# Spockuto/drand

Hardware: AMD Instinct MI355X
Metric: beacons verified/s (batch chain verify) (higher is better)
Workload: dtype u32 (381-bit Montgomery, 12x32-bit limbs); 1 GPU; configs[1]: 1000000-round chained beacon history per GPU, chain.VerifyBeacon per round; beacons_per_gpu=1000000, segment_len=64, parallelism=range-shard x1

## Files before the change

### drand_amd/_lib.py

```python
from __future__ import annotations

import ctypes
import os

_HERE = os.path.dirname(os.path.abspath(__file__))
LIB_PATH = os.environ.get("DRAND_AMD_LIB", os.path.join(_HERE, "libblsverify.so"))

BLSV_OK = 0
BLSV_EINVAL = -1
BLSV_EHIP = -2
BLSV_ENOGROUP = -3
BLSV_ENOTENOUGH = -4

AGG_OK = 0
AGG_OK_V2 = 1
AGG_V1_RECOVER_FAIL = 2
AGG_V1_INVALID = 3
AGG_V2_RECOVER_FAIL = 4

REJ_OK = 0
REJ_LENGTH = 1
REJ_FLAG = 2
REJ_INF_NONZERO = 3
REJ_X_GE_P = 4
REJ_NOT_ON_CURVE = 5
REJ_NOT_IN_SUBGROUP = 6
REJ_PAIRING = 7
REJ_SHARE_INDEX = 8

REJ_NAMES = {
    REJ_OK: "ok",
    REJ_LENGTH: "bad length",
    REJ_FLAG: "bad compression flag",
    REJ_INF_NONZERO: "infinity with non-zero bits",
    REJ_X_GE_P: "coordinate >= p",
    REJ_NOT_ON_CURVE: "point is not on curve",
    REJ_NOT_IN_SUBGROUP: "point is not on correct subgroup",
    REJ_PAIRING: "bls: invalid signature",
    REJ_SHARE_INDEX: "tbls: invalid signature share",
}

u8p = ctypes.POINTER(ctypes.c_uint8)
u32p = ctypes.POINTER(ctypes.c_uint32)
u64p = ctypes.POINTER(ctypes.c_uint64)
vp = ctypes.c_void_p
sz = ctypes.c_size_t

SIGNATURES = {
    "blsv_version": (ctypes.c_char_p, []),
    "blsv_device_count": (ctypes.c_int, []),
    "blsv_create": (ctypes.c_int, [ctypes.c_int, ctypes.POINTER(vp)]),
    "blsv_destroy": (None, [vp]),
    "blsv_last_error": (ctypes.c_char_p, [vp]),
    "blsv_synchronize": (ctypes.c_int, [vp]),
    "blsv_set_group": (ctypes.c_int, [vp, u8p, sz, sz]),
    "blsv_verify_chained": (ctypes.c_int, [vp, ctypes.c_uint64, u8p, sz, u8p, sz, u8p, u64p, u8p]),
    "blsv_verify_chained_multi": (ctypes.c_int, [ctypes.POINTER(vp), sz, ctypes.POINTER(sz), ctypes.c_uint64, u8p, sz,
                                                  u8p, sz, u8p, u64p, u8p]),
    "blsv_verify_prevs": (ctypes.c_int, [vp, ctypes.c_uint64, u8p, sz, u8p, sz, u8p, u64p, u8p]),
    "blsv_verify_unchained": (ctypes.c_int, [vp, u64p, ctypes.c_uint64, u8p, sz, u8p, u64p, u8p]),
    "blsv_verify_messages": (ctypes.c_int, [vp, u8p, u8p, u32p, sz, u8p, u8p, u64p, u8p]),
    "blsv_verify_partials": (ctypes.c_int, [vp, u8p, sz, u8p, sz, sz, u8p, u8p]),
    "blsv_verify_partials_multi": (ctypes.c_int, [vp, u8p, u32p, u8p, sz, sz, u8p, u8p]),
    "blsv_recover": (ctypes.c_int, [vp, u8p, sz, u8p, sz, sz, sz, sz, u8p]),
    "blsv_aggregate": (ctypes.c_int, [vp, u8p, sz, u8p, sz, sz, sz, sz, u8p, u8p, u8p, u8p]),
    "blsv_aggregate_round": (ctypes.c_int, [vp, u8p, sz, u8p, sz, u8p, sz, u8p, sz, sz, sz, sz, u8p, u8p, u8p, u8p,
                                             ctypes.POINTER(ctypes.c_int32), u8p]),
    "blsv_sign": (ctypes.c_int, [vp, u8p, ctypes.c_int32, u8p, u32p, sz, u8p]),
    "blsv_verify_chained_dev": (ctypes.c_int, [vp, ctypes.c_uint64, ctypes.c_uint64, ctypes.c_uint64, vp, sz, vp, sz,
                                                vp, vp, vp, vp]),
    "blsv_generate_chained_dev": (ctypes.c_int, [vp, u8p, ctypes.c_uint64, ctypes.c_uint64, vp, sz, vp, sz, vp]),
    "blsv_profile_enable": (ctypes.c_int, [vp, ctypes.c_int]),
    "blsv_profile_read": (ctypes.c_int, [vp, ctypes.POINTER(ctypes.c_double), u64p, u64p, ctypes.c_int]),
    "blsv_lat_trace": (ctypes.c_int, [vp, u64p, ctypes.c_int, ctypes.POINTER(ctypes.c_double), ctypes.c_int]),
    "blsv_test_fp_mul": (ctypes.c_int, [vp, u32p, u32p, sz, u32p]),
    "blsv_test_op": (ctypes.c_int, [vp, ctypes.c_char_p, u32p, sz, u32p]),
    "blsv_test_op_info": (ctypes.c_int, [ctypes.c_int, ctypes.POINTER(ctypes.c_char_p), ctypes.POINTER(ctypes.c_int),
                                         ctypes.POINTER(ctypes.c_int), ctypes.POINTER(ctypes.c_int)]),
    "blsv_test_pairing": (ctypes.c_int, [vp, u32p, u32p, sz, u32p]),
    "blsv_test_hash_to_g2": (ctypes.c_int, [vp, u8p, u32p, sz, u32p, u8p]),
    "blsv_test_final_exp": (ctypes.c_int, [vp, u32p, sz, u32p, u32p]),
    "blsv_test_tail_split": (ctypes.c_int, [vp, sz]),
    "blsv_set_lat_max": (sz, [vp, sz]),
    "blsv_set_chunk": (sz, [vp, sz]),
    "blsv_workspace_bytes": (sz, [vp]),
    "blsv_lat_trace_enable": (ctypes.c_int, [vp, ctypes.c_int]),
    "blsv_test_generic_chains": (ctypes.c_int, [vp, ctypes.c_int]),
    "blsv_test_spec_stats": (ctypes.c_int, [vp, ctypes.POINTER(ctypes.c_uint64), ctypes.POINTER(ctypes.c_uint64)]),
    "blsv_test_lagrange": (ctypes.c_int, [ctypes.POINTER(ctypes.c_uint32), ctypes.c_size_t, ctypes.POINTER(ctypes.c_uint32)]),
    "blsv_service_create": (ctypes.c_int, [ctypes.c_int, ctypes.c_uint32, ctypes.c_uint32, ctypes.POINTER(vp)]),
    "blsv_service_destroy": (None, [vp]),
    "blsv_service_verify_partial": (ctypes.c_int, [vp, u8p, sz, sz, u8p, sz, u8p, sz, u8p, u8p]),
    "blsv_service_verify_recovered": (ctypes.c_int, [vp, u8p, u8p, sz, u8p, u8p, u8p]),
    "blsv_service_stats": (ctypes.c_int, [vp, u64p, u64p, u64p]),
    "blsv_test_service_limits": (ctypes.c_int, [vp, sz, sz, sz, u64p]),
    "blsv_verify_chained_rlc": (ctypes.c_int, [vp, ctypes.c_uint64, u8p, sz, u8p, sz, u8p, u64p, u8p]),
    "blsv_verify_unchained_rlc": (ctypes.c_int, [vp, u64p, ctypes.c_uint64, u8p, sz, u8p, u64p, u8p]),
    "blsv_verify_chained_rlc_dev": (ctypes.c_int, [vp, ctypes.c_uint64, ctypes.c_uint64, ctypes.c_uint64, vp, sz, vp,
                                                    sz, vp, vp, vp, vp]),
    "blsv_set_rlc_group": (sz, [vp, sz]),
    "blsv_rlc_stats": (ctypes.c_int, [vp, u64p, u64p, u64p]),
    "blsv_test_rlc_seed": (ctypes.c_int, [vp, u8p]),
    "blsv_test_rlc_sums": (ctypes.c_int, [vp, ctypes.c_uint64, u8p, sz, u8p, sz, u8p, u8p]),
    "blsv_tlock_open": (ctypes.c_int, [vp, u8p, u8p, sz, u8p, u8p, u8p, u8p]),
    "blsv_tlock_open_dev": (ctypes.c_int, [vp, u8p, vp, sz, vp, vp, vp]),
    "blsv_tlock_stats": (ctypes.c_int, [vp, u64p, u64p]),
    "blsv_tlock_seal": (ctypes.c_int, [vp, u8p, ctypes.c_uint64, u8p, sz, u8p, u8p, u8p]),
    "blsv_tlock_seal_dev": (ctypes.c_int, [vp, u8p, ctypes.c_uint64, vp, sz, vp, vp, vp, vp]),
    "blsv_tlock_seal_stats": (ctypes.c_int, [vp, u64p, u64p]),
}

_lib = None


class EngineUnavailable(RuntimeError):
    """The HIP engine library could not be loaded (no silent fallback exists)."""


def load():
    global _lib
    if _lib is not None:
        return _lib
    if not os.path.exists(LIB_PATH):
        raise EngineUnavailable(
            f"{LIB_PATH} not found: build it with `python -c 'import __graft_entry__ as g; g.build()'` "
            "(make -C drand_amd/csrc); drand_amd has no CPU fallback")
    try:
        lib = ctypes.CDLL(LIB_PATH)
    except OSError as e:
        raise EngineUnavailable(f"cannot load {LIB_PATH}: {e}") from e
    for name, (res, args) in SIGNATURES.items():
        fn = getattr(lib, name)
        fn.restype = res
        fn.argtypes = args
    _lib = lib
    return lib


def buf(data):
    if data is None:
        return None
    b = bytes(data)
    arr = (ctypes.c_uint8 * max(len(b), 1)).from_buffer_copy(b if b else b"\0")
    return arr


def out_buf(n):
    return (ctypes.c_uint8 * max(n, 1))()
```

### drand_amd/csrc/blsverify.cpp

```cpp
#include "host_internal.h"

void release_workspace(blsv_ctx* c) {
  for (DBuf* d : {&c->H, &c->HQ, &c->S, &c->F, &c->FW, &c->LN, &c->h_inf, &c->s_inf, &c->cls}) d->release();
  c->cap = 0;
}

int ensure_workspace(blsv_ctx* c, size_t cnt) {
  for (;;) {
    size_t want = std::min(std::max(cnt, size_t(64)), c->chunk);
    want = (want + 63) & ~size_t(63);
    if (want <= c->cap) return BLSV_OK;
    hipError_t e = hipSuccess;
    auto need = [&](DBuf& d, size_t bytes) {
      if (e == hipSuccess) e = d.ensure(bytes);
    };
    need(c->H, want * blsk::H_WORDS * 4);
    need(c->HQ, kHqWords(want) * 4);
    need(c->S, want * blsk::S_WORDS * 4);
    need(c->F, want * blsk::F_WORDS * 4);
    need(c->FW, 3 * want * blsk::F_WORDS * 4);
    need(c->LN, std::max(std::min(want, kLineSub) * blsk::MILLER_LINE_WORDS, blsk::FEXP_PARK_WORDS(want)) * 4);
    need(c->h_inf, want);
    need(c->s_inf, want);
    need(c->cls, want);
    static_assert(3 * blsk::F_WORDS >= 48 * 64 / 21 + 1, "FW holds the Miller park of a sub-chunk");
    if (e == hipSuccess) {
      c->cap = want;
      return BLSV_OK;
    }
    release_workspace(c);
    (void)hipGetLastError();
    if (e != hipErrorOutOfMemory || want <= kMinChunk)
      return fail(c, BLSV_EHIP, "staging for %zu items: %s", want, hipGetErrorString(e));
    c->chunk = std::max(kMinChunk, ((want / 2) + 63) & ~size_t(63));
    c->lat_max = std::min(c->lat_max, c->chunk);
    c->oom_halvings++;
  }
}

hipError_t h2d(blsv_ctx* c, void* dst, const void* src, size_t len) {
  if (!len) return hipSuccess;
  if (len > kIoCap / 4) return hipMemcpyAsync(dst, src, len, hipMemcpyHostToDevice, c->stream);
  if (!c->io_up.p) {
    hipError_t e = c->io_up.ensure(kIoCap);
    if (e != hipSuccess) return e;
  }
  if (c->io_up_off + len > kIoCap) {
    hipError_t e = hipStreamSynchronize(c->stream);
    if (e != hipSuccess) return e;
    c->io_up_off = 0;
  }
  uint8_t* h = c->io_up.as<uint8_t>() + c->io_up_off;
  memcpy(h, src, len);
  c->io_up_off += (len + 63) & ~size_t(63);
  return hipMemcpyAsync(dst, h, len, hipMemcpyHostToDevice, c->stream);
}

hipError_t download_sync(blsv_ctx* c, std::initializer_list<Down> ds) {
  size_t total = 0;
  for (const Down& d : ds) total += (d.len + 63) & ~size_t(63);
  const bool staged = total <= kIoCap && (c->io_down.p || c->io_down.ensure(kIoCap) == hipSuccess);
  hipError_t e = hipSuccess;
  size_t off = 0;
  for (const Down& d : ds) {
    if (!d.len) continue;
    void* to = staged ? (void*)(c->io_down.as<uint8_t>() + off) : d.user;
    if (e == hipSuccess) e = hipMemcpyAsync(to, d.dev, d.len, hipMemcpyDeviceToHost, c->stream);
    off += (d.len + 63) & ~size_t(63);
  }
  const hipError_t es = hipStreamSynchronize(c->stream);
  if (e == hipSuccess) e = es;
  if (e == hipSuccess) c->io_up_off = 0;
  if (e != hipSuccess || !staged) return e;
  off = 0;
  for (const Down& d : ds) {
    if (d.len) memcpy(d.user, c->io_down.as<uint8_t>() + off, d.len);
    off += (d.len + 63) & ~size_t(63);
  }
  return hipSuccess;
}

hipEvent_t take_event(blsv_ctx* c) {
  if (!c->event_pool.empty()) {
    hipEvent_t e = c->event_pool.back();
    c->event_pool.pop_back();
    return e;
  }
  hipEvent_t e = nullptr;
  if (hipEventCreate(&e) != hipSuccess) return nullptr;
  return e;
}

extern "C" {

const char* blsv_version(void) { return "drand_amd blsverify 0.1 (gfx950)"; }

int blsv_device_count(void) {
  int n = 0;
  return hipGetDeviceCount(&n) == hipSuccess ? n : 0;
}

int blsv_create(int device, blsv_ctx** out) {
  if (!out) return BLSV_EINVAL;
  *out = nullptr;
  blsv_ctx* c = new blsv_ctx();
  c->device = device;
  hipError_t e = hipSetDevice(device);
  if (e == hipSuccess) e = hipStreamCreateWithFlags(&c->stream, hipStreamNonBlocking);
  if (e == hipSuccess) e = hipStreamCreateWithFlags(&c->side, hipStreamNonBlocking);
  if (e == hipSuccess) e = hipStreamCreateWithFlags(&c->side2, hipStreamNonBlocking);
  for (hipEvent_t& ev : c->hash_ev)
    if (e == hipSuccess) e = hipEventCreateWithFlags(&ev, hipEventDisableTiming);
  if (e == hipSuccess) e = hipEventCreateWithFlags(&c->fork_ev, hipEventDisableTiming);
  if (e == hipSuccess) e = hipEventCreateWithFlags(&c->join_ev, hipEventDisableTiming);
  int cus = 0;
  if (e == hipSuccess) e = hipDeviceGetAttribute(&cus, hipDeviceAttributeMultiprocessorCount, device);
  c->tail_q_dev = c->tail_q = size_t(64) * 4 * (size_t)std::max(cus, 0);
  if (e != hipSuccess) {
    fprintf(stderr, "blsv_create: %s\n", hipGetErrorString(e));
    blsv_destroy(c);
    return BLSV_EHIP;
  }
  *out = c;
  return BLSV_OK;
}

void blsv_destroy(blsv_ctx* c) {
  if (!c) return;
  (void)hipSetDevice(c->device);
  for (hipStream_t s : {c->stream, c->side, c->side2}) {
    if (!s) continue;
    (void)hipStreamSynchronize(s);
    (void)hipStreamDestroy(s);
  }
  for (hipEvent_t ev : c->hash_ev)
    if (ev) (void)hipEventDestroy(ev);
  if (c->fork_ev) (void)hipEventDestroy(c->fork_ev);
  if (c->join_ev) (void)hipEventDestroy(c->join_ev);
  (void)hipDeviceSynchronize();
  for (auto& r : c->recs)
    for (hipEvent_t e : {r.a, r.b, r.a2, r.b2})
      if (e) (void)hipEventDestroy(e);
  for (auto e : c->event_pool) (void)hipEventDestroy(e);
  delete c;
}

const char* blsv_last_error(const blsv_ctx* c) { return c ? c->err.c_str() : "null context"; }

int blsv_synchronize(blsv_ctx* c) {
  if (!c) return BLSV_EINVAL;
  HIPCHK(c, hipStreamSynchronize(c->stream));
  return BLSV_OK;
}

int blsv_profile_enable(blsv_ctx* c, int on) {
  if (!c) return BLSV_EINVAL;
  c->prof = on != 0;
  return BLSV_OK;
}

int blsv_profile_read(blsv_ctx* c, double* ms, uint64_t* launches, uint64_t* items, int nstages) {
  if (!c || nstages < 0) return BLSV_EINVAL;
  (void)hipSetDevice(c->device);
  for (int s = 0; s < nstages; s++) {
    if (ms) ms[s] = 0;
    if (launches) launches[s] = 0;
    if (items) items[s] = 0;
  }
  for (auto& r : c->recs) {
    HIPCHK(c, hipEventSynchronize(r.b));
    float t = 0;
    HIPCHK(c, hipEventElapsedTime(&t, r.a, r.b));
    if (r.a2 && r.b2) {
      float t2 = 0;
      HIPCHK(c, hipEventSynchronize(r.b2));
      HIPCHK(c, hipEventElapsedTime(&t2, r.a2, r.b2));
      t += t2;
    }
    if (r.stage < nstages) {
      if (ms) ms[r.stage] += t;
      if (launches) launches[r.stage] += 1;
      if (items) items[r.stage] += r.items;
    }
    for (hipEvent_t e : {r.a, r.b, r.a2, r.b2})
      if (e) c->event_pool.push_back(e);
  }
  c->recs.clear();
  return ST_N;
}

size_t blsv_set_lat_max(blsv_ctx* c, size_t lat_max) {
  if (!c) return 0;
  const size_t prev = c->lat_max;
  c->lat_max = std::min(lat_max, c->chunk);
  return prev;
}

size_t blsv_set_chunk(blsv_ctx* c, size_t items) {
  if (!c) return 0;
  const size_t prev = c->chunk;
  size_t v = items ? std::min(std::max(items, kMinChunk), kMaxChunk) : chunk_env();
  v = (v + 63) & ~size_t(63);
  (void)hipSetDevice(c->device);
  if (v < c->cap) {
    (void)hipStreamSynchronize(c->stream);
    (void)hipStreamSynchronize(c->side);
    release_workspace(c);
  }
  c->chunk = v;
  c->lat_max = std::min(c->lat_max, v);
  return prev;
}

size_t blsv_workspace_bytes(const blsv_ctx* c) {
  if (!c) return 0;
  size_t b = 0;
  for (const DBuf* d : {&c->H, &c->HQ, &c->S, &c->F, &c->FW, &c->LN, &c->h_inf, &c->s_inf, &c->cls}) b += d->sz;
  return b;
}

}
```

### drand_amd/csrc/engine_ctx.h

```cpp
#pragma once
#include <hip/hip_runtime.h>

#include <algorithm>
#include <cerrno>
#include <cstdarg>
#include <cstdio>
#include <cstdlib>
#include <cstring>
#include <string>
#include <vector>

#include "../../include/blsverify.h"
#include "kernels.h"

namespace blsv_detail {

constexpr size_t kMaxChunk = size_t(1) << 20;
constexpr size_t kMinChunk = size_t(1) << 14;
constexpr size_t kLineSub = kMaxChunk;
constexpr size_t kPkTable = 4096;
constexpr size_t kFexpParkWords(size_t items) { return blsk::FEXP_PARK_WORDS(items) + 48 * 64; }
constexpr size_t kHqWords(size_t items) { return std::max(items * blsk::HQ_WORDS, kFexpParkWords(items)); }
constexpr size_t kStagingBytesPerItem =
    4 * (blsk::H_WORDS + blsk::HQ_WORDS + 3 + blsk::S_WORDS + 4 * blsk::F_WORDS + blsk::MILLER_LINE_WORDS) + 3;
// ... 2 lines not shown
static_assert((133ull * kMaxChunk) * 4 < 0xffffffffull, "SoA VGPR byte offset exceeds 32 bits");
static_assert(48ull * 4 * kMaxChunk < 0x7fffffffull, "3-lane park slot resource exceeds 31 bits");
static_assert(blsk::G1_WORDS <= blsk::H_WORDS, "timelock: the U table does not fit the H staging");
static_assert(blsk::F_WORDS <= blsk::HQ_WORDS, "timelock: the captured Fp12 does not fit the HQ staging");
static_assert(BLSV_GT_LEN == 4 * blsk::F_WORDS, "timelock: the Gt encoding is one F staging row per item");
static_assert(BLSV_U_LEN <= 4 * blsk::S_WORDS, "timelock: a host call's compressed U bytes do not fit the S staging");
static_assert(BLSV_SCALAR_LEN <= 4 * blsk::S_WORDS, "sealing: a host call's scalars do not fit the S staging");
static_assert(BLSV_U_LEN <= 4 * blsk::H_WORDS, "sealing: the compressed U bytes do not fit the H staging");
static_assert(blsk::G1_WORDS <= blsk::S_WORDS, "sealing: the decoded key does not fit the S staging");
static_assert(blsk::FEXP_PARK_WORDS(1) + blsk::kTlockTabWords <= 64 * blsk::MILLER_LINE_WORDS,
              "sealing: the base's line table does not fit LN behind the park (the smallest workspace is 64 items)");

struct DBuf {
  void* p = nullptr;
  size_t sz = 0;
  ~DBuf() {
    if (p) (void)hipFree(p);
  }
  void release() {
    if (p) (void)hipFree(p);
    p = nullptr;
    sz = 0;
  }
  hipError_t ensure(size_t need) {
    if (need <= sz) return hipSuccess;
    if (p) {
      (void)hipFree(p);
      p = nullptr;
      sz = 0;
    }
    size_t want = std::max(need, size_t(256));
    hipError_t e = hipMalloc(&p, want);
    if (e == hipSuccess) sz = want;
    return e;
  }
  template <typename T>
  T* as() const {
    return static_cast<T*>(p);
  }
};

struct PinBuf {
  void* p = nullptr;
  size_t sz = 0;
  ~PinBuf() {
    if (p) (void)hipHostFree(p);
  }
  hipError_t ensure(size_t need) {
    if (need <= sz) return hipSuccess;
    if (p) (void)hipHostFree(p);
    p = nullptr;
    sz = 0;
    const size_t want = std::max(need + need / 2, size_t(4096));
    hipError_t e = hipHostMalloc(&p, want, hipHostMallocDefault);
    if (e == hipSuccess) sz = want;
    return e;
  }
  template <typename T>
  T* as() const {
    return static_cast<T*>(p);
  }
};

}
using namespace blsv_detail;

enum Stage {
  ST_HASH = 0,
  ST_DECOMP = 1,
  ST_MILLER = 2,
  ST_FEXP = 3,
  ST_FINISH = 4,
  ST_LAT = 5,
  ST_RLC = 6,
  ST_TLOCK = 7,
  ST_N = 8
};
struct ProfRec {
  int stage;
  size_t items;
  hipEvent_t a, b;
  hipEvent_t a2 = nullptr, b2 = nullptr;
};

constexpr size_t kRlcGroupDefault = 64;
constexpr size_t kRlcGroupMin = 8, kRlcGroupMax = 4096;
constexpr size_t kLatMaxDefault = 1536;
inline size_t chunk_env() {
  static const size_t v = [] {
    const char* e = getenv("BLSV_CHUNK");
    if (!e) return kMaxChunk;
    char* end = nullptr;
    errno = 0;
    const unsigned long long x = strtoull(e, &end, 10);
    if (end == e || *end != '\0' || errno == ERANGE || e[0] == '-' || x == 0) {
      fprintf(stderr, "blsverify: ignoring BLSV_CHUNK=\"%s\" (not a positive integer); chunk stays %zu\n", e, kMaxChunk);
      return kMaxChunk;
    }
    const size_t c = (size_t)std::min<unsigned long long>(std::max<unsigned long long>(x, kMinChunk), kMaxChunk);
    return (c + 63) & ~size_t(63);
  }();
  return v;
}

inline size_t lat_max_env() {
  static const size_t v = [] {
    const char* e = getenv("BLSV_LAT_MAX");
    if (!e) return kLatMaxDefault;
    char* end = nullptr;
    errno = 0;
    const unsigned long long x = strtoull(e, &end, 10);
    if (end == e || *end != '\0' || errno == ERANGE || e[0] == '-') {
      fprintf(stderr, "blsverify: ignoring BLSV_LAT_MAX=\"%s\" (not a non-negative integer); cutover stays %zu\n", e,
              kLatMaxDefault);
      return kLatMaxDefault;
    }
    return (size_t)std::min<unsigned long long>(x, kMaxChunk);
  }();
  return v;
}

struct rlc_state {
  size_t group = kRlcGroupDefault;
  bool seed_pinned = false;
  uint8_t seed[32] = {0};
  uint64_t groups = 0, groups_failed = 0, items_exact = 0;
  DBuf part, gH, gS, g_hinf, g_sinf, gcls, cH, cS, c_hinf, c_sinf, ccls, fail, out96;
  PinBuf host;
};

struct tlock_state {
  bool valid = false;
  uint8_t sig[96] = {0};
  uint8_t cls = 0;
  uint64_t prepared = 0, items = 0;
  DBuf d_sig, S, s_inf, s_cls, tab;
};

struct tseal_state {
  bool valid = false, t1_built = false;
  uint8_t pk[48] = {0};
  uint64_t round = 0;
  uint64_t bases = 0, items = 0;
  DBuf t1, t2;
};

struct blsv_ctx {
  int device = 0;
  bool prof = false;
  size_t chunk = chunk_env();
  size_t lat_max = std::min(lat_max_env(), chunk);
  uint64_t oom_halvings = 0;
  size_t tail_q_dev = 0, tail_q = 0;
  std::vector<ProfRec> recs;
  std::vector<hipEvent_t> event_pool;
  hipStream_t stream = nullptr;
  hipStream_t side = nullptr;
  hipEvent_t fork_ev = nullptr, join_ev = nullptr;
  hipStream_t side2 = nullptr;
  hipEvent_t hash_ev[2] = {nullptr, nullptr};
  std::string err;
  bool has_group = false;
  size_t t = 0, n = 0;
  DBuf commits, commit_inf;
  std::vector<uint8_t> group_bytes;
  DBuf pk_all, pk_all_inf;
  size_t pk_all_n = 0;
  bool pk_all_built = false;
  DBuf pk_tab, pk_inf;
  uint8_t pk_cache[48];
  bool pk_cache_valid = false;
  size_t cap = 0;
  DBuf H, S, F, FW, LN, h_inf, s_inf, cls;
  DBuf HQ;
  DBuf in_sigs, in_msgs, in_off, in_len, in_rounds, seeds, bitmap, first_bad, sk, idx, lambdas, scratch, out,
      pp_tab, pp_inf, sel, g1_cls, misc;
  PinBuf pin;
  PinBuf io_up, io_down;
  size_t io_up_off = 0;
  struct SpecSlot {
    DBuf sig, S, s_inf, cls, sel, lam, scratch, out, vmsg, voff, vlen, vcls;
    DBuf hout, saff;
    PinBuf host;
  } spec[2];
  uint64_t spec_hits = 0, spec_misses = 0;
  DBuf arena;
  rlc_state rlc;
  tlock_state tlock;
  tseal_state tseal;
};

#define HIPCHK(ctx, expr)                                                             \
  do {                                                                                \
    hipError_t e_ = (expr);                                                           \
    if (e_ != hipSuccess) return fail((ctx), BLSV_EHIP, "%s: %s", #expr, hipGetErrorString(e_)); \
  } while (0)

inline int fail(blsv_ctx* ctx, int code, const char* fmt, ...) {
  char buf[512];
  va_list ap;
  va_start(ap, fmt);
  vsnprintf(buf, sizeof buf, fmt, ap);
  va_end(ap);
  if (ctx) ctx->err = buf;
  return code;
}


int ensure_workspace(blsv_ctx* c, size_t cnt);
void release_workspace(blsv_ctx* c);

int svc_verify_mixed(blsv_ctx* c, size_t n, const uint8_t* msgs, const uint64_t* off, const uint32_t* lens,
                     const uint8_t* sigs96, const uint32_t* idx, const uint32_t* d_tab, const uint8_t* d_tab_inf,
                     uint8_t* cls_out);
```

### drand_amd/csrc/fp.h

```cpp
#pragma once
#include <stdint.h>
#include "bls_constants.h"

#ifdef BLS_HOST
#include <stddef.h>
#define DI inline
#define NOINL static inline
namespace bls {
extern unsigned long long g_fp_mul_count;
}
#define BLS_COUNT_MUL() (++::bls::g_fp_mul_count)
#else
#include <hip/hip_runtime.h>
#define DI __device__ __forceinline__
#define NOINL static __device__ __noinline__
#define BLS_COUNT_MUL() ((void)0)
#endif

namespace bls {

struct fp {
  uint32_t l[12];
};

// ... 603 lines not shown

DI fp fp_pow_sqrt_inv(const fp& a) { return fp_from_u12(fp_pow_p_minus_3_div_4(fp_to_u12(a))); }


DI int fp_bitlen12(const uint32_t (&c)[12]) {
  int n = 0;
#pragma unroll
  for (int i = 0; i < 12; i++) n = c[i] ? 32 * i + 32 - __builtin_clz(c[i]) : n;
  return n;
}

DI uint64_t fp_top33(const uint32_t (&x)[12], int s) {
  const int w = s >> 5, o = s & 31;
  uint32_t x0 = 0, x1 = 0;
#pragma unroll
  for (int i = 0; i < 12; i++) {
    x0 = i == w ? x[i] : x0;
    x1 = i == w + 1 ? x[i] : x1;
  }
  return ((((uint64_t)x1 << 32) | x0) >> o) & ((1ull << 33) - 1);
}

DI int64_t fp_lincomb28(const uint32_t (&X)[14], const uint32_t (&Y)[14], int64_t f, int64_t g,
                        uint32_t (&L)[14]) {
  int64_t acc = 0;
#pragma unroll
  for (int k = 0; k < 14; k++) {
    acc += (int64_t)X[k] * f + (int64_t)Y[k] * g;
    L[k] = (uint32_t)acc & M28;
    acc >>= 28;
  }
  return acc;
}

DI void fp_lincomb_shr31(const uint32_t (&X)[14], const uint32_t (&Y)[14], int64_t f, int64_t g, uint32_t (&r)[12],
                         bool& neg) {
  uint32_t L[16];
  uint32_t L14[14];
  const int64_t top = fp_lincomb28(X, Y, f, g, L14);
#pragma unroll
  for (int k = 0; k < 14; k++) L[k] = L14[k];
  L[14] = (uint32_t)top & M28;
  L[15] = (uint32_t)(top >> 28) & M28;
#pragma unroll
  for (int j = 0; j < 12; j++) {
    const int B = 31 + 32 * j, k = B / 28, o = B % 28;
    uint64_t v = ((uint64_t)L[k] >> o) | ((uint64_t)L[k + 1] << (28 - o));
    if (k + 2 < 16) v |= (uint64_t)L[k + 2] << (56 - o);
    r[j] = (uint32_t)v;
  }
  neg = top < 0;
  const uint32_t m = neg ? 0xffffffffu : 0u;
  unsigned c = neg ? 1u : 0u;
#pragma unroll
  for (int j = 0; j < 12; j++) r[j] = __builtin_addc(r[j] ^ m, 0u, c, &c);
}

DI fp fp_lincomb_mont56(const uint32_t (&X)[14], const uint32_t (&Y)[14], int64_t f, int64_t g) {
  uint32_t m[2], L[14];
  int64_t acc = 0;
#pragma unroll
  for (int k = 0; k < 16; k++) {
    if (k < 14) acc += (int64_t)X[k] * f + (int64_t)Y[k] * g;
#pragma unroll
    for (int j = 0; j < 2; j++)
      if (j < k && k - j < 14) acc += (int64_t)m[j] * P28[k - j];
    if (k < 2) {
      m[k] = ((uint32_t)acc * P_INV28) & M28;
      acc += (int64_t)m[k] * P28[0];
      acc >>= 28;
    } else {
      L[k - 2] = (uint32_t)acc & M28;
      acc >>= 28;
    }
  }
  const u12 w = fp_join28(L);
  const uint32_t msk = acc < 0 ? 0xffffffffu : 0u;
  fp r;
  unsigned c = 0;
#pragma unroll
  for (int i = 0; i < 12; i++) r.l[i] = __builtin_addc(w[i], P2_RAW[i] & msk, c, &c);
  return r;
}

DI u12 fp_inv_bingcd_raw(u12 yin, bool& converged) {
  uint32_t a[12], b[12];
  const fp yc = fp_canon(fp_from_u12(yin));
#pragma unroll
  for (int i = 0; i < 12; i++) {
    a[i] = yc.l[i];
    b[i] = P_RAW[i];
  }
  fp u = fp_zero(), v = fp_zero();
  u.l[0] = 1;
#pragma unroll 1
  for (int it = 0; it < 25; it++) {
    uint32_t c[12];
#pragma unroll
    for (int i = 0; i < 12; i++) c[i] = a[i] | b[i];
    const int n0 = fp_bitlen12(c), n = n0 > 64 ? n0 : 64;
    uint64_t A = ((uint64_t)(a[0] & 0x7fffffffu)) | (fp_top33(a, n - 33) << 31);
    uint64_t B = ((uint64_t)(b[0] & 0x7fffffffu)) | (fp_top33(b, n - 33) << 31);
    int64_t f0 = 1, g0 = 0, f1 = 0, g1 = 1;
#pragma unroll
    for (int j = 0; j < 31; j++) {
      const bool odd = (A & 1u) != 0;
      const bool sw = odd & (A < B);
      const uint64_t A2 = sw ? B : A, B2 = sw ? A : B;
      const int64_t F0 = sw ? f1 : f0, G0 = sw ? g1 : g0, F1 = sw ? f0 : f1, G1 = sw ? g0 : g1;
      A = odd ? A2 - B2 : A2;
      f0 = odd ? F0 - F1 : F0;
      g0 = odd ? G0 - G1 : G0;
      B = B2;
      f1 = F1;
      g1 = G1;
      A >>= 1;
      f1 = (int64_t)((uint64_t)f1 << 1);
      g1 = (int64_t)((uint64_t)g1 << 1);
    }
    uint32_t X[14], Y[14];
    u12 av, bv;
#pragma unroll
    for (int i = 0; i < 12; i++) av[i] = a[i], bv[i] = b[i];
    fp_split28(av, X);
    fp_split28(bv, Y);
    bool na, nb;
    fp_lincomb_shr31(X, Y, f0, g0, a, na);
    fp_lincomb_shr31(X, Y, f1, g1, b, nb);
    f0 = na ? -f0 : f0;
    g0 = na ? -g0 : g0;
    f1 = nb ? -f1 : f1;
    g1 = nb ? -g1 : g1;
    fp_split28(fp_to_u12(u), X);
    fp_split28(fp_to_u12(v), Y);
    u = fp_lincomb_mont56(X, Y, f0, g0);
    v = fp_lincomb_mont56(X, Y, f1, g1);
  }
  uint32_t nb = b[0] ^ 1u;
#pragma unroll
  for (int i = 1; i < 12; i++) nb |= b[i];
  converged = (nb == 0) | fp_raw_is_zero(yc);
  return fp_to_u12(fp_mul(v, fp_load_const(FP_INV_FIX)));
}

NOINL u12 fp_inv_bingcd(u12 yin) {
  bool ok;
  u12 r = fp_inv_bingcd_raw(yin, ok);
  if (!ok) r = fp_pow_p_minus_2(yin);
  return r;
}

DI fp fp_inv(const fp& a) { return fp_from_u12(fp_inv_bingcd(fp_to_u12(a))); }

DI fp fp_sqrt_cand(const fp& a) { return fp_from_u12(fp_pow_sqrt(fp_to_u12(a))); }

DI bool fp_is_square(const fp& a) {
  fp l = fp_from_u12(fp_pow_legendre(fp_to_u12(a)));
  return fp_is_zero(l) || fp_eq(l, fp_one());
}

DI fp fp_raw_from_be48(const uint8_t* b) {
  fp r;
#pragma unroll
  for (int i = 0; i < 12; i++) {
    const uint8_t* q = b + 44 - 4 * i;
    r.l[i] = ((uint32_t)q[0] << 24) | ((uint32_t)q[1] << 16) | ((uint32_t)q[2] << 8) | (uint32_t)q[3];
  }
  return r;
}

DI void fp_raw_to_be48(uint8_t* b, const fp& a) {
#pragma unroll
  for (int i = 0; i < 12; i++) {
    uint8_t* q = b + 44 - 4 * i;
    q[0] = (uint8_t)(a.l[i] >> 24);
    q[1] = (uint8_t)(a.l[i] >> 16);
    q[2] = (uint8_t)(a.l[i] >> 8);
    q[3] = (uint8_t)a.l[i];
  }
}

DI bool fp_raw_lt_p(const fp& a) {
  unsigned br = 0;
#pragma unroll
  for (int i = 0; i < 12; i++) (void)__builtin_subc(a.l[i], P_RAW[i], br, &br);
  return br != 0;
}

DI bool fp_raw_gt_half(const fp& a) {
  unsigned br = 0;
#pragma unroll
  for (int i = 0; i < 12; i++) (void)__builtin_subc(FP_P_MINUS_1_DIV_2_RAW[i], a.l[i], br, &br);
  return br != 0;
}

DI bool fp_mont_is_odd(const fp& a) { return fp_from_mont(a).l[0] & 1u; }

}
```

### drand_amd/csrc/host_internal.h

```cpp
#pragma once
#include <functional>
#include <initializer_list>

#include "engine_ctx.h"
#include "hostlogic.h"

#pragma GCC visibility push(hidden)

constexpr size_t kIoCap = size_t(1) << 20;
hipError_t h2d(blsv_ctx* c, void* dst, const void* src, size_t len);
struct Down {
  void* user;
  const void* dev;
  size_t len;
};
hipError_t download_sync(blsv_ctx* c, std::initializer_list<Down> ds);

hipEvent_t take_event(blsv_ctx* c);
struct StageTimer {
  blsv_ctx* c;
  int stage;
  size_t items;
  hipStream_t st;
  hipEvent_t a = nullptr;
  StageTimer(blsv_ctx* c_, int stage_, size_t items_, hipStream_t st_) : c(c_), stage(stage_), items(items_), st(st_) {
    if (c->prof && (a = take_event(c))) (void)hipEventRecord(a, st);
  }
  ~StageTimer() {
    if (!a) return;
    hipEvent_t b = take_event(c);
    if (!b) return;
    (void)hipEventRecord(b, st);
    c->recs.push_back({stage, items, a, b});
  }
};

struct Staging {
  uint32_t *H, *HQ, *S, *F, *FW, *LN;
  uint8_t *h_inf, *s_inf, *cls;
};
inline Staging staging(const blsv_ctx* c) {
  return {c->H.as<uint32_t>(),    c->HQ.as<uint32_t>(),   c->S.as<uint32_t>(),
          c->F.as<uint32_t>(),    c->FW.as<uint32_t>(),   c->LN.as<uint32_t>(),
          c->h_inf.as<uint8_t>(), c->s_inf.as<uint8_t>(), c->cls.as<uint8_t>()};
}

struct SigSrc {
  const uint8_t* d;
  size_t stride, offset;
};
struct PkSel {
  const uint32_t* tab;
  const uint8_t* inf;
  const uint32_t* idx;
};
inline PkSel group_pk(const blsv_ctx* c) { return {c->commits.as<uint32_t>(), c->commit_inf.as<uint8_t>(), nullptr}; }

inline void hash_chained(blsv_ctx* c, const blsk::ChainedSrc& src, size_t base, size_t cnt, hipStream_t st) {
  const Staging w = staging(c);
  blsk::launch_hash_chained(src, base, cnt, w.H, w.h_inf, w.HQ, st);
}
inline void hash_messages(blsv_ctx* c, const uint8_t* d_msgs, const uint64_t* d_off, const uint32_t* d_len, size_t base,
                          size_t cnt, hipStream_t st) {
  const Staging w = staging(c);
  blsk::launch_hash_messages(d_msgs, d_off + base, d_len + base, cnt, w.H, w.h_inf, w.HQ, st);
}
inline void hash_uploaded(blsv_ctx* c, size_t base, size_t cnt, hipStream_t st) {
  hash_messages(c, c->in_msgs.as<uint8_t>(), c->in_off.as<uint64_t>(), c->in_len.as<uint32_t>(), base, cnt, st);
}
inline void lat_uploaded(blsv_ctx* c, const SigSrc& sig, size_t cnt, const PkSel& pk, uint8_t* cls, uint32_t* S,
                         uint8_t* s_inf, hipStream_t st) {
  blsk::launch_lat_messages(c->in_msgs.as<uint8_t>(), c->in_off.as<uint64_t>(), c->in_len.as<uint32_t>(), sig.d,
                            sig.stride, sig.offset, cnt, pk.tab, pk.inf, pk.idx, cls, S, s_inf, st);
}
inline void final_exp(blsv_ctx* c, size_t cnt, size_t base, size_t m, uint8_t* cls, hipStream_t st,
                      uint32_t* out = nullptr) {
  const Staging w = staging(c);
  blsk::launch_final_exp(w.F, w.FW, cnt, base, m, cls, st, w.HQ + (base ? blsk::FEXP_PARK_WORDS(base) : 0), out);
}
inline void final_exp(blsv_ctx* c, size_t cnt, uint8_t* cls, hipStream_t st, uint32_t* out = nullptr) {
  final_exp(c, cnt, 0, cnt, cls, st, out);
}

inline bool use_lat(const blsv_ctx* c, size_t n) { return n > 0 && n <= std::min(c->lat_max, c->cap); }
inline bool use_rlc(const blsv_ctx* c, size_t n) { return n > c->lat_max && n >= 2 * c->rlc.group; }

template <typename F>
inline int for_each_pass(const blsv_ctx* c, size_t n, F f) {
  for (size_t base = 0; base < n; base += c->cap) {
    const int rc = f(base, std::min(c->cap, n - base));
    if (rc) return rc;
  }
  return BLSV_OK;
}

using HashFn = std::function<void(size_t base, size_t cnt, hipStream_t st)>;
struct Tail {
  bool randomized = false;
  uint32_t seed[8] = {0};
  bool fused_subgroup() const { return !randomized; }
};
struct PassOut {
  uint64_t* bitmap;
  unsigned long long* first_bad;
  uint8_t* cls;
  uint64_t label0;
};
int run_head(blsv_ctx* c, const SigSrc& sig, size_t base, size_t cnt, const Tail& tail, hipStream_t st,
             const HashFn& hash);
int run_passes(blsv_ctx* c, size_t n, const SigSrc& sig, const PkSel& pk, const HashFn& hash, const Tail& tail,
               const PassOut& out, hipStream_t st);
int ctx_outputs(blsv_ctx* c, size_t n, bool with_cls, PassOut& out);

int rlc_draw_seed(blsv_ctx* c, uint32_t (&w)[8]);
int rlc_sums(blsv_ctx* c, size_t base, size_t cnt, const uint32_t (&seed)[8], hipStream_t st);

int stage_chain(blsv_ctx* c, uint64_t first_round, const uint8_t* prevs, size_t prev0_len, bool prev_rows,
                const uint8_t* sigs96, size_t n, blsk::ChainedSrc& src);
int decode_g1(blsv_ctx* c, const uint8_t* pk48, size_t cnt, DBuf& tab, DBuf& inf, std::vector<uint8_t>& cls);
int upload_messages(blsv_ctx* c, const uint8_t* msgs, const uint32_t* msg_lens, size_t n);

#pragma GCC visibility pop
```

### drand_amd/csrc/k_fexp.hip

```cpp
#include "kcommon.h"

namespace blsk {

BLS_KERNEL(BLS_WPE_FEXP) k_fexp_easy(const uint32_t* F, size_t n, size_t m, const uint8_t* cls, uint32_t* G) {
  size_t i = (size_t)blockIdx.x * TPB + threadIdx.x;
  if (i >= m || cls[i] != REJ_OK) return;
  st_fp12(G, n, i, fexp_easy(ld_fp12(F, n, i)));
}

#ifndef BLS_WPE_FEXP_TRI
#define BLS_WPE_FEXP_TRI 2
#endif

struct TriPark {
  uint32_t* p;
  size_t n, i;
};

template <typename LoadX>
DI fp4 tri_pow_x_abs(const tri_lane& t, LoadX lx, const TriPark& pk) {
  constexpr uint64_t NSQ = 1ull | (2ull << 6) | (3ull << 12) | (9ull << 18) | (32ull << 24) | (16ull << 30);
  fp4 r = lx();
#pragma unroll 1
  for (int s = 0; s < 6; s++) {
    const int n = (int)((NSQ >> (6 * s)) & 63u);
#pragma unroll 1
    for (int k = 0; k < n; k++) r = tri_cyclotomic_sqr(t, r);
    if (s < 5) r = tri_mul_lp(t, r, lx(), pk.p, pk.n, pk.i);
  }
  return r;
}

template <int MODE>
BLS_KERNEL(BLS_WPE_FEXP_TRI) k_fexp_tri(const uint32_t* X, const uint32_t* C, const uint32_t* G, size_t n, size_t m,
                                        uint8_t* cls, uint32_t* OUT, uint32_t* park) {
  const tri_lane t = tri_lane_id();
#if BLS_CSQR_LIN
  kp_lds_init<11>();
#endif
  const size_t ir = (size_t)blockIdx.x * TRI_GROUPS + t.group;
  const bool in_range = t.group < TRI_GROUPS && ir < m;
  const size_t i0 = in_range ? ir : m - 1;
  const bool live = in_range && cls[i0] == REJ_OK;
  const TriPark pk = {park, (size_t)gridDim.x * TPB, (size_t)blockIdx.x * TPB + t.lane};
  auto at = [&](const uint32_t* B) {
    size_t j = i0;
    asm volatile("" : "+v"(j));
    return tri_load(B, n, j, t.role);
  };
  fp4 r = tri_conj(t, tri_pow_x_abs(t, [&]() { return at(X); }, pk));
  if (MODE == 0 || MODE == 1) r = tri_mul_lp(t, r, tri_conj(t, at(X)), pk.p, pk.n, pk.i);
  if (MODE == 2) r = tri_mul_lp(t, r, tri_frob(t, at(X)), pk.p, pk.n, pk.i);
  if (MODE == 4) {
    r = tri_mul_lp(t, r, tri_frob2(t, at(C)), pk.p, pk.n, pk.i);
    r = tri_mul_lp(t, r, tri_conj(t, at(C)), pk.p, pk.n, pk.i);
    r = tri_mul_lp(t, r, tri_cyclotomic_sqr(t, at(G)), pk.p, pk.n, pk.i);
    r = tri_mul_lp(t, r, at(G), pk.p, pk.n, pk.i);
  }
  if (MODE < 4 || OUT) {
    if (live) tri_store(OUT, n, i0, t.role, r);
  }
  if (MODE == 4) {
    const bool one = tri_is_one(t, r);
    if (live && t.role == 0 && !one) cls[i0] = REJ_PAIRING;
  }
}

void launch_final_exp(uint32_t* F, uint32_t* W, size_t n, size_t base, size_t m, uint8_t* cls, hipStream_t st,
                      uint32_t* park, uint32_t* out) {
  if (!m) return;
  F += base;
  cls += base;
  if (out) out += base;
  uint32_t* G = W + base;
  uint32_t* B = G + n * F_WORDS;
  uint32_t* C = G + 2 * n * F_WORDS;
  const dim3 grid(grid_for(m)), blk(TPB);
  hipLaunchKernelGGL(k_fexp_easy, grid, blk, 0, st, F, n, m, cls, G);
  const dim3 tgrid((unsigned)((m + TRI_GROUPS - 1) / TRI_GROUPS));
  hipLaunchKernelGGL(k_fexp_tri<0>, tgrid, blk, 0, st, G, nullptr, nullptr, n, m, cls, F, park);
  hipLaunchKernelGGL(k_fexp_tri<1>, tgrid, blk, 0, st, F, nullptr, nullptr, n, m, cls, B, park);
  hipLaunchKernelGGL(k_fexp_tri<2>, tgrid, blk, 0, st, B, nullptr, nullptr, n, m, cls, C, park);
  hipLaunchKernelGGL(k_fexp_tri<3>, tgrid, blk, 0, st, C, nullptr, nullptr, n, m, cls, F, park);
  hipLaunchKernelGGL(k_fexp_tri<4>, tgrid, blk, 0, st, F, C, G, n, m, cls, out, park);
}

}
```

### drand_amd/csrc/k_hash.hip

```cpp
#define BLS_FP2_KARA_INL 1
#ifndef BLS_G2_DBL_KARA
#define BLS_G2_DBL_KARA 0
#endif
#include "kcommon.h"

namespace blsk {

__constant__ uint8_t c_dst[DST_LEN] = {66, 76, 83, 95, 83, 73, 71, 95, 66, 76, 83, 49, 50, 51, 56, 49, 71, 50, 95, 88, 77, 68,
                                       58, 83, 72, 65, 45, 50, 53, 54, 95, 83, 83, 87, 85, 95, 82, 79, 95, 78, 85, 76, 95};

DI void store_h(uint32_t* H, uint8_t* h_inf, size_t cnt, size_t i, const g2j& h) {
  bool inf = jac_is_inf(h);
  g2a a = g2_to_aff(h);
  st_fp2(H, cnt, i, 0, a.x);
  st_fp2(H, cnt, i, 2, a.y);
  h_inf[i] = inf;
}

DI g2j load_jac(const uint32_t* Q, size_t cnt, size_t i, int slot) {
  return {ld_fp2(Q, cnt, i, slot), ld_fp2(Q, cnt, i, slot + 2), ld_fp2(Q, cnt, i, slot + 4)};
}
DI void store_jac(uint32_t* Q, size_t cnt, size_t i, int slot, const g2j& p) {
  st_fp2(Q, cnt, i, slot, p.x);
  st_fp2(Q, cnt, i, slot + 2, p.y);
// ... 22 lines not shown
  }
}

template <bool SPLIT>
DI void hash_a_index(int& k, size_t& i) {
  k = SPLIT ? (int)(blockIdx.x & 1u) : 0;
  i = (size_t)(SPLIT ? blockIdx.x >> 1 : blockIdx.x) * TPB + threadIdx.x;
}

template <bool SPLIT>
BLS_KERNEL(BLS_WPE_HASH_A) k_hash_chained(ChainedSrc src, size_t base, size_t cnt, uint32_t* Q) {
  int k;
  size_t i;
  hash_a_index<SPLIT>(k, i);
  if (i >= cnt) return;
  const size_t g = base + i;
  const size_t seg = (g + src.seg_phase) / src.seg_len;
  const bool seg_start = g == 0 || (g + src.seg_phase - seg * src.seg_len) == 0;
  const uint8_t* prev;
  int prev_len;
  if (seg_start) {
    prev = src.seeds + seg * 96;
    prev_len = seg == 0 ? (int)src.seed0_len : 96;
  } else {
    prev = src.sigs + (g - 1) * 96;
    prev_len = 96;
  }
  uint32_t msg[8];
  drand_message<BLS_SHA_FAST_BATCH>(msg, prev, prev_len, src.first_round + g);
  fp2 u0, u1;
  hash_to_field_fp2(msg, u0, u1);
  hash_a_store<SPLIT>(u0, u1, k, Q, cnt, i);
}

template <bool SPLIT>
BLS_KERNEL(BLS_WPE_HASH_A) k_hash_unchained(const uint64_t* rounds, uint64_t first_round, size_t base,
                                            size_t cnt, uint32_t* Q) {
  int k;
  size_t i;
  hash_a_index<SPLIT>(k, i);
  if (i >= cnt) return;
  const uint64_t round = rounds ? rounds[base + i] : first_round + base + i;
  uint32_t msg[8];
  drand_message_v2<BLS_SHA_FAST_BATCH>(msg, round);
  fp2 u0, u1;
  hash_to_field_fp2(msg, u0, u1);
  hash_a_store<SPLIT>(u0, u1, k, Q, cnt, i);
}

template <bool SPLIT>
BLS_KERNEL(BLS_WPE_HASH_A) k_hash_messages(const uint8_t* msgs, const uint64_t* off, const uint32_t* len,
                                           size_t cnt, uint32_t* Q) {
  int k;
  size_t i;
  hash_a_index<SPLIT>(k, i);
  if (i >= cnt) return;
  uint32_t b0[8];
  xmd_b0_bytes<BLS_SHA_FAST_BATCH>(b0, msgs + off[i], len[i], c_dst);
  fp2 u0, u1;
  xmd_tail_to_field(b0, u0, u1);
  hash_a_store<SPLIT>(u0, u1, k, Q, cnt, i);
}

enum : uint8_t { COF_LOAD, COF_STORE, COF_DBL, COF_ADD, COF_NEG, COF_PSI2, COF_CHECK, COF_END };
constexpr uint8_t COF_NEGY = 1, COF_PSI = 2;
struct CofOp {
  uint8_t op, arg, flags, pad;
};
#define COF_CHAIN(s)                                                                                  \
  {COF_DBL, 1, 0, 0}, {COF_ADD, s, 0, 0}, {COF_DBL, 2, 0, 0}, {COF_ADD, s, 0, 0}, {COF_DBL, 3, 0, 0}, \
      {COF_ADD, s, 0, 0}, {COF_DBL, 9, 0, 0}, {COF_ADD, s, 0, 0}, {COF_DBL, 32, 0, 0}, {COF_ADD, s, 0, 0}, \
      {COF_DBL, 16, 0, 0}
__constant__ CofOp c_cof_prog[] = {
    {COF_LOAD, 0, 0, 0}, {COF_ADD, 6, 0, 0}, {COF_CHECK, 0, 0, 0}, {COF_STORE, 0, 0, 0},
    COF_CHAIN(0), {COF_NEG, 0, 0, 0}, {COF_ADD, 0, COF_PSI, 0}, {COF_STORE, 6, 0, 0},
    COF_CHAIN(6), {COF_NEG, 0, 0, 0}, {COF_ADD, 6, COF_NEGY, 0}, {COF_STORE, 6, 0, 0},
    {COF_LOAD, 0, 0, 0}, {COF_DBL, 1, 0, 0}, {COF_PSI2, 0, 0, 0}, {COF_ADD, 0, COF_NEGY, 0},
    {COF_ADD, 6, 0, 0}, {COF_STORE, 6, 0, 0}, {COF_END, 0, 0, 0}};
#undef COF_CHAIN

BLS_KERNEL(BLS_WPE_HASH_B) k_hash_cofactor(uint32_t* Q, size_t cnt, uint8_t* redo) {
  size_t i = (size_t)blockIdx.x * TPB + threadIdx.x;
  if (i >= cnt) return;
  auto ld = [&](int slot) {
    size_t j = i;
    asm volatile("" : "+v"(j));
    return ld_fp2(Q, cnt, j, slot);
  };
  __shared__ uint4 park_lds[18 * TPB];
  const LdsFp2Slots park = {park_lds};
  g2j acc = {};
  bool exc = false;
#pragma unroll 1
  for (int pc = 0;; pc++) {
    const CofOp o = c_cof_prog[pc];
    if (o.op == COF_END) break;
    const int s = o.arg;
    if (o.op == COF_LOAD) {
      acc = {ld(s), ld(s + 2), ld(s + 4)};
    } else if (o.op == COF_STORE) {
      store_jac(Q, cnt, i, s, acc);
    } else if (o.op == COF_DBL) {
#pragma unroll 1
      for (int k = 0; k < s; k++) acc = g2_dbl_inl(acc);
    } else if (o.op == COF_ADD) {
      const bool psi = o.flags & COF_PSI, negy = o.flags & COF_NEGY;
      acc = g2_add_inl_exc(
          acc,
          [&]() {
            const fp2 x = ld(s);
            return psi ? fp2_mul_inl(fp2_conj(x), fp2_load_const(PSI_KX)) : x;
          },
          [&]() {
            fp2 y = ld(s + 2);
            if (psi) y = fp2_mul_inl(fp2_conj(y), fp2_load_const(PSI_KY));
            return negy ? fp2_neg(y) : y;
          },
          [&]() {
            const fp2 z = ld(s + 4);
            return psi ? fp2_conj(z) : z;
          },
          park, exc);
    } else if (o.op == COF_NEG) {
      acc.y = fp2_neg(acc.y);
    } else if (o.op == COF_PSI2) {
      const fp kx = fp_load_const(PSI2_KX[0]), ky = fp_load_const(PSI2_KY[0]);
      acc.x = {fp_mul_inl(acc.x.c0, kx), fp_mul_inl(acc.x.c1, kx)};
      acc.y = {fp_mul_inl(acc.y.c0, ky), fp_mul_inl(acc.y.c1, ky)};
    } else if (o.op == COF_CHECK) {
      if (exc) {
        redo[i] = 2;
        return;
      }
    }
  }
  redo[i] = exc;
}

BLS_KERNEL(BLS_WPE_HASH_B) k_hash_cofactor_generic(uint32_t* Q, size_t cnt, const uint8_t* redo, int all) {
  size_t i = (size_t)blockIdx.x * TPB + threadIdx.x;
  if (i >= cnt) return;
  const uint8_t rd = redo[i];
  if (!(all || rd)) return;
  if (rd == 2) store_jac(Q, cnt, i, 0, jac_add(load_jac(Q, cnt, i, 0), load_jac(Q, cnt, i, 6)));
  store_jac(Q, cnt, i, 6, g2_clear_cofactor_reload([&]() { return load_jac(Q, cnt, i, 0); }));
}

BLS_KERNEL(BLS_WPE_HASH_C) k_hash_affine(const uint32_t* Q, size_t cnt, uint32_t* H, uint8_t* h_inf) {
  size_t i = (size_t)blockIdx.x * TPB + threadIdx.x;
  if (i >= cnt) return;
  store_h(H, h_inf, cnt, i, load_jac(Q, cnt, i, 6));
}

int g_generic_chains_all = 0;
static void launch_hash_bc(uint32_t* Q, size_t cnt, uint32_t* H, uint8_t* h_inf, hipStream_t st) {
  hipLaunchKernelGGL(k_hash_cofactor, dim3(grid_for(cnt)), dim3(TPB), 0, st, Q, cnt, h_inf);
  hipLaunchKernelGGL(k_hash_cofactor_generic, dim3(grid_for(cnt)), dim3(TPB), 0, st, Q, cnt, h_inf,
                     g_generic_chains_all);
  hipLaunchKernelGGL(k_hash_affine, dim3(grid_for(cnt)), dim3(TPB), 0, st, Q, cnt, H, h_inf);
}

#ifndef BLS_HASH_SPLIT_MAX
#define BLS_HASH_SPLIT_MAX 65536
#endif
static inline dim3 hash_a_grid(size_t cnt, bool split) { return dim3((split ? 2u : 1u) * grid_for(cnt)); }

void launch_hash_chained(const ChainedSrc& src, size_t base, size_t cnt, uint32_t* H, uint8_t* h_inf,
                         uint32_t* Q, hipStream_t st) {
  if (!cnt) return;
  const bool split = cnt <= BLS_HASH_SPLIT_MAX;
  if (split)
    hipLaunchKernelGGL(k_hash_chained<true>, hash_a_grid(cnt, true), dim3(TPB), 0, st, src, base, cnt, Q);
  else
    hipLaunchKernelGGL(k_hash_chained<false>, hash_a_grid(cnt, false), dim3(TPB), 0, st, src, base, cnt, Q);
  launch_hash_bc(Q, cnt, H, h_inf, st);
}

void launch_hash_unchained(const uint64_t* rounds, uint64_t first_round, size_t base, size_t cnt, uint32_t* H,
                           uint8_t* h_inf, uint32_t* Q, hipStream_t st) {
  if (!cnt) return;
  const bool split = cnt <= BLS_HASH_SPLIT_MAX;
  if (split)
    hipLaunchKernelGGL(k_hash_unchained<true>, hash_a_grid(cnt, true), dim3(TPB), 0, st, rounds, first_round, base,
                       cnt, Q);
  else
    hipLaunchKernelGGL(k_hash_unchained<false>, hash_a_grid(cnt, false), dim3(TPB), 0, st, rounds, first_round, base,
                       cnt, Q);
  launch_hash_bc(Q, cnt, H, h_inf, st);
}

void launch_hash_messages(const uint8_t* msgs, const uint64_t* off, const uint32_t* len, size_t cnt, uint32_t* H,
                          uint8_t* h_inf, uint32_t* Q, hipStream_t st) {
  if (!cnt) return;
  const bool split = cnt <= BLS_HASH_SPLIT_MAX;
  if (split)
    hipLaunchKernelGGL(k_hash_messages<true>, hash_a_grid(cnt, true), dim3(TPB), 0, st, msgs, off, len, cnt, Q);
  else
    hipLaunchKernelGGL(k_hash_messages<false>, hash_a_grid(cnt, false), dim3(TPB), 0, st, msgs, off, len, cnt, Q);
  launch_hash_bc(Q, cnt, H, h_inf, st);
}

}
```

### drand_amd/csrc/kernels.h

```cpp
#pragma once
#include <hip/hip_runtime.h>
#include <stddef.h>
#include <stdint.h>

namespace blsk {

constexpr int H_WORDS = 48;
constexpr int S_WORDS = 48;
constexpr int F_WORDS = 144;
constexpr int G1_WORDS = 24;

struct ChainedSrc {
  const uint8_t* sigs;
  const uint8_t* seeds;
  uint64_t first_round;
  uint64_t seg_len;
  uint32_t seed0_len;
  uint64_t seg_phase;
};

constexpr int HQ_WORDS = 144;
void launch_hash_chained(const ChainedSrc& src, size_t base, size_t cnt, uint32_t* H, uint8_t* h_inf,
                         uint32_t* Q, hipStream_t st);
void launch_hash_unchained(const uint64_t* rounds, uint64_t first_round, size_t base, size_t cnt, uint32_t* H,
                           uint8_t* h_inf, uint32_t* Q, hipStream_t st);
void launch_hash_messages(const uint8_t* msgs, const uint64_t* off, const uint32_t* len, size_t cnt,
                          uint32_t* H, uint8_t* h_inf, uint32_t* Q, hipStream_t st);
void launch_decompress_g2(const uint8_t* sigs, size_t stride, size_t offset, size_t base, size_t cnt, uint32_t* S,
                          uint8_t* s_inf, uint8_t* cls, hipStream_t st);
constexpr int MILLER_LINE_WORDS = 68 * 2 * 6 * 12;
void launch_miller(const uint32_t* pk_tab, const uint8_t* pk_inf, const uint32_t* pk_idx, const uint32_t* H,
                   const uint8_t* h_inf, const uint32_t* S, const uint8_t* s_inf, uint8_t* cls, size_t cnt,
                   uint32_t* F, uint32_t* LN, size_t sub, uint32_t* park, bool check_subgroup, hipStream_t st);
void launch_miller_lines(const uint32_t* pk_tab, const uint8_t* pk_inf, const uint32_t* pk_idx, const uint32_t* H,
                         const uint8_t* h_inf, const uint32_t* S, const uint8_t* s_inf, uint8_t* cls, size_t cnt,
                         size_t base, size_t m, uint32_t* LN, size_t sub, bool check_subgroup, hipStream_t st);
void launch_miller_f(const uint32_t* LN, size_t sub, const uint8_t* cls, size_t cnt, size_t base, size_t m,
                     uint32_t* F, uint32_t* park, bool single_lane, hipStream_t st);
constexpr size_t TRI_PARK_WORDS(size_t items) { return 48 * 64 * ((items + 20) / 21); }
constexpr size_t FEXP_PARK_WORDS(size_t items) { return TRI_PARK_WORDS(items); }
void launch_final_exp(uint32_t* F, uint32_t* W, size_t n, size_t base, size_t m, uint8_t* cls, hipStream_t st,
                      uint32_t* park, uint32_t* out = nullptr);
void launch_finish(const uint8_t* cls, size_t base, size_t cnt, uint64_t* bitmap, unsigned long long* first_bad,
                   uint64_t label0, hipStream_t st);

constexpr size_t kRlcLaneItems = 8;
constexpr size_t kRlcPartWords = 72;
constexpr size_t rlc_lanes(size_t cnt) { return (cnt + kRlcLaneItems - 1) / kRlcLaneItems; }
constexpr size_t rlc_groups(size_t cnt, size_t group) { return (cnt + group - 1) / group; }
void launch_rlc_sums(const uint32_t* H, const uint8_t* h_inf, const uint32_t* S, const uint8_t* s_inf,
                     const uint8_t* cls, size_t cnt, uint64_t index0, const uint32_t* seed_words, size_t group,
                     uint32_t* part, uint32_t* GH, uint8_t* g_hinf, uint32_t* GS, uint8_t* g_sinf, hipStream_t st);
void launch_rlc_gather(const uint32_t* fail, size_t group, size_t m, const uint32_t* H, const uint8_t* h_inf,
                       const uint32_t* S, const uint8_t* s_inf, const uint8_t* cls, size_t cnt, uint32_t* CH,
                       uint8_t* c_hinf, uint32_t* CS, uint8_t* c_sinf, uint8_t* ccls, hipStream_t st);
void launch_rlc_scatter(const uint32_t* fail, size_t group, size_t m, const uint8_t* ccls, uint8_t* cls, size_t cnt,
                        hipStream_t st);
void launch_rlc_compress(const uint32_t* GP, const uint8_t* g_inf, size_t ng, uint8_t* out96, hipStream_t st);

constexpr size_t kTlockTabWords = 68 * 3 * 24;
void launch_tlock_prepare(const uint32_t* S, const uint8_t* s_inf, const uint8_t* s_cls, uint32_t* tab, hipStream_t st);
void launch_tlock_f(const uint32_t* tab, const uint32_t* U, const uint8_t* u_inf, const uint8_t* cls,
                    const uint8_t* sig_inf, size_t cnt, uint32_t* F, hipStream_t st);
void launch_tlock_encode(const uint32_t* E, const uint8_t* cls, size_t cnt, uint8_t* out, hipStream_t st);

constexpr size_t kTsealT1Words = 64 * 15 * 24;
constexpr size_t kTsealT2Words = 64 * 15 * 144;
void launch_tseal_g1_table(uint32_t* T1, hipStream_t st);
void launch_tseal_gt_table(const uint32_t* B, uint32_t* T2, hipStream_t st);
void launch_tseal_u(const uint32_t* T1, const uint8_t* scalars, size_t cnt, uint8_t* us, uint8_t* ok, uint8_t* cls,
                    hipStream_t st);
void launch_tseal_gt(const uint32_t* T2, const uint8_t* scalars, const uint8_t* cls, size_t cnt, uint32_t* E,
                     hipStream_t st);

int lat_trace_read(uint64_t* out, int n, hipStream_t st);
int lat_trace_clear(hipStream_t st);
int lat_trace_enable(int on, hipStream_t st);
extern int g_generic_chains_all;
void launch_lat_chained(const ChainedSrc& src, size_t base, size_t cnt, const uint32_t* pk_tab, const uint8_t* pk_inf,
                        uint8_t* cls, hipStream_t st);
void launch_lat_unchained(const uint64_t* rounds, uint64_t first_round, const uint8_t* sigs, size_t base, size_t cnt,
                          const uint32_t* pk_tab, const uint8_t* pk_inf, uint8_t* cls, hipStream_t st);
void launch_lat_messages(const uint8_t* msgs, const uint64_t* off, const uint32_t* len, const uint8_t* sigs,
                         size_t stride, size_t offset, size_t cnt, const uint32_t* pk_tab, const uint8_t* pk_inf,
                         const uint32_t* pk_idx, uint8_t* cls, uint32_t* S, uint8_t* s_inf, hipStream_t st);

void launch_decompress_g1(const uint8_t* in, size_t cnt, uint32_t* tab, uint8_t* inf, uint8_t* cls, hipStream_t st);
void launch_pubpoly_eval(const uint32_t* commits, const uint8_t* commit_inf, uint32_t t, const uint32_t* idx,
                         size_t cnt, uint32_t* out_tab, uint8_t* out_inf, hipStream_t st);
void launch_lat_decode(const uint8_t* sigs, size_t stride, size_t offset, size_t cnt, uint32_t* S, uint8_t* s_inf,
                       uint8_t* cls, hipStream_t st);
void launch_decompress_g2_only(const uint8_t* sigs, size_t stride, size_t offset, size_t base, size_t cnt,
                               uint32_t* S, uint8_t* s_inf, uint8_t* cls, hipStream_t st);
void launch_lat_recover(const uint32_t* S, size_t n_s, const uint8_t* s_inf, const uint32_t* sel,
                        const uint32_t* lambdas, uint32_t t, uint32_t* scratch, uint8_t* out96, hipStream_t st,
                        uint32_t* saff = nullptr);
constexpr size_t kLatHoutWords = 448, kLatSaffWords = 192;
void launch_lat_hash_key(const uint8_t* msgs, const uint64_t* off, const uint32_t* len, const uint32_t* pk_tab,
                         const uint8_t* pk_inf, uint32_t* hout, hipStream_t st);
void launch_lat_verify_pre(const uint32_t* hout, const uint32_t* saff, uint8_t* cls, hipStream_t st);
void launch_sign(const uint32_t* sk_words, int32_t index, const uint32_t* H, const uint8_t* h_inf, size_t cnt,
                 uint8_t* out, size_t out_stride, hipStream_t st);
void launch_gen_chained(const uint32_t* sk_words, const ChainedSrc& src, size_t n, uint8_t* sigs_out, hipStream_t st);

bool launch_test_op(int op, const uint32_t* in, size_t cnt, uint32_t* out, uint32_t* park, hipStream_t st);
bool launch_test_op_mf(int op, const uint32_t* in, size_t cnt, uint32_t* out, hipStream_t st);
void launch_test_fp_mul(const uint32_t* a, const uint32_t* b, size_t cnt, uint32_t* out, hipStream_t st);
void launch_test_pairing(const uint32_t* p_tab, const uint32_t* q_aff, size_t cnt, uint32_t* out_f, hipStream_t st);
void launch_test_unpack_g2(const uint32_t* H, size_t cnt, uint32_t* out, hipStream_t st);
void launch_test_pack_fp12(const uint32_t* f, size_t cnt, uint32_t* F, hipStream_t st);
void launch_test_unpack_fp12(const uint32_t* F, size_t cnt, uint32_t* out, hipStream_t st);
void launch_test_final_exp_ref(const uint32_t* F, size_t cnt, uint32_t* out, hipStream_t st);

}
```

### drand_amd/csrc/pairing.h

```cpp
#pragma once
#include "curve.h"

namespace bls {

struct g2proj {
  fp2 x, y, z;
};

DI fp2 fp2_mul_3b(const fp2& c) {
  fp2 x4 = fp2_dbl(fp2_dbl(fp2_mul_xi(c)));
  return fp2_add(fp2_dbl(x4), x4);
}

template <bool INL = false>
DI void miller_dbl_step(g2proj& t, fp2& l00, fp2& l01, fp2& l11, const fp& xp, const fp& yp) {
  auto mul = [](const fp2& a, const fp2& b) { return INL ? fp2_mul_inl(a, b) : fp2_mul(a, b); };
  auto sqr = [](const fp2& a) { return INL ? fp2_sqr_inl(a) : fp2_sqr(a); };
  fp2 A = fp2_half(mul(t.x, t.y));
  fp2 B = sqr(t.y);
  fp2 C = sqr(t.z);
  fp2 E = fp2_mul_3b(C);
  fp2 F = fp2_mul3(E);
  fp2 G = fp2_half(fp2_add(B, F));
  fp2 H = fp2_sub(sqr(fp2_add_lazy(t.y, t.z)), fp2_add(B, C));
// ... 98 lines not shown
  }
  return ok;
}

template <typename Put, typename XP, typename YP>
DI void miller_dbl_step_inl(g2proj& t, Put put, XP xp, YP yp) {
  miller_dbl_step_ts(g2proj_reg{t}, put, xp, yp);
}
template <typename Put, typename Q, typename XP, typename YP>
DI void miller_add_step_inl(g2proj& t, Q qload, Put put, XP xp, YP yp) {
  miller_add_step_ts(g2proj_reg{t}, qload, put, xp, yp);
}

DI void miller_add_step(g2proj& t, const g2a& q, fp2& l00, fp2& l01, fp2& l11, const fp& xp, const fp& yp) {
  fp2 theta = fp2_sub(t.y, fp2_mul(q.y, t.z));
  fp2 delta = fp2_sub(t.x, fp2_mul(q.x, t.z));
  l00 = fp2_sub(fp2_mul(theta, q.x), fp2_mul(delta, q.y));
  l01 = fp2_neg(fp2_mul_fp(theta, xp));
  l11 = fp2_mul_fp(delta, yp);
  fp2 C = fp2_sqr(theta);
  fp2 D = fp2_sqr(delta);
  fp2 E = fp2_mul(D, delta);
  fp2 F = fp2_mul(t.z, C);
  fp2 G = fp2_mul(t.x, D);
  fp2 H = fp2_sub(fp2_add(E, F), fp2_dbl(G));
  t.x = fp2_mul(delta, H);
  t.y = fp2_sub(fp2_mul(theta, fp2_sub(G, H)), fp2_mul(t.y, E));
  t.z = fp2_mul(t.z, E);
}

struct line {
  fp2 a0, a1, a4;
};

DI fp12 line_mul_line(const line& a, const line& b) {
  fp2 t00 = fp2_mul(a.a0, b.a0), t11 = fp2_mul(a.a1, b.a1), t44 = fp2_mul(a.a4, b.a4);
  fp2 c01 = fp2_sub(fp2_sub(fp2_mul(fp2_add_lazy(a.a0, a.a1), fp2_add_lazy(b.a0, b.a1)), t00), t11);
  fp2 c11 = fp2_sub(fp2_sub(fp2_mul(fp2_add_lazy(a.a0, a.a4), fp2_add_lazy(b.a0, b.a4)), t00), t44);
  fp2 c12 = fp2_sub(fp2_sub(fp2_mul(fp2_add_lazy(a.a1, a.a4), fp2_add_lazy(b.a1, b.a4)), t11), t44);
  return {{fp2_add(t00, fp2_mul_xi(t44)), c01, t11}, {fp2_zero(), c11, c12}};
}

DI fp6 fp6_mul_by_12(const fp6& a, const fp2& b1, const fp2& b2) {
  fp2 t1 = fp2_mul(a.c1, b1), t2 = fp2_mul(a.c2, b2);
  fp2 m = fp2_sub(fp2_sub(fp2_mul(fp2_add_lazy(a.c1, a.c2), fp2_add_lazy(b1, b2)), t1), t2);
  return {fp2_mul_xi(m), fp2_add(fp2_mul(a.c0, b1), fp2_mul_xi(t2)), fp2_add(fp2_mul(a.c0, b2), t1)};
}

DI fp12 fp12_mul_by_line_pair(const fp12& f, const fp12& L) {
  fp6 t0 = fp6_mul(f.c0, L.c0);
  fp6 t1 = fp6_mul_by_12(f.c1, L.c1.c1, L.c1.c2);
  fp6 Ls = {L.c0.c0, fp2_add_lazy(L.c0.c1, L.c1.c1), fp2_add_lazy(L.c0.c2, L.c1.c2)};
  fp6 c1 = fp6_sub(fp6_sub(fp6_mul(fp6_add_lazy(f.c0, f.c1), Ls), t0), t1);
  return {fp6_add(t0, fp6_mul_v(t1)), c1};
}

DI line line_one() { return {fp2_one(), fp2_zero(), fp2_zero()}; }

DI fp12 miller_loop_2(const g1a (&P)[2], const g2a (&Q)[2], const bool (&active)[2]) {
  g2proj T[2];
#pragma unroll
  for (int k = 0; k < 2; k++) T[k] = {Q[k].x, Q[k].y, fp2_one()};
  fp12 f = fp12_one();
  bool first = true;
#pragma unroll 1
  for (int i = 62; i >= 0; i--) {
    if (!first) f = fp12_sqr(f);
    line l[2];
#pragma unroll
    for (int k = 0; k < 2; k++) {
      miller_dbl_step(T[k], l[k].a0, l[k].a1, l[k].a4, P[k].x, P[k].y);
      if (!active[k]) l[k] = line_one();
    }
    f = first ? line_mul_line(l[0], l[1]) : fp12_mul_by_line_pair(f, line_mul_line(l[0], l[1]));
    first = false;
    if ((BLS_X_ABS >> i) & 1ull) {
#pragma unroll
      for (int k = 0; k < 2; k++) {
        miller_add_step(T[k], Q[k], l[k].a0, l[k].a1, l[k].a4, P[k].x, P[k].y);
        if (!active[k]) l[k] = line_one();
      }
      f = fp12_mul_by_line_pair(f, line_mul_line(l[0], l[1]));
    }
  }
  return fp12_conj(f);
}

constexpr int MILLER_STEPS = 68;

template <typename LoadQ, typename Emit>
DI void miller_lines(const g1a& P, LoadQ load_q, Emit emit) {
  const g2a Q0 = load_q();
  g2proj T = {Q0.x, Q0.y, fp2_one()};
  int step = 0;
#pragma unroll 1
  for (int i = 62; i >= 0; i--) {
    line l;
    miller_dbl_step<false>(T, l.a0, l.a1, l.a4, P.x, P.y);
    emit(step++, l);
    if ((BLS_X_ABS >> i) & 1ull) {
      miller_add_step(T, load_q(), l.a0, l.a1, l.a4, P.x, P.y);
      emit(step++, l);
    }
  }
}

template <typename LoadLine>
DI fp12 miller_f_from_lines(LoadLine load) {
  fp12 f = fp12_one();
  int step = 0;
#pragma unroll 1
  for (int i = 62; i >= 0; i--) {
    if (i != 62) f = fp12_sqr(f);
    const fp12 L = line_mul_line(load(step, 0), load(step, 1));
    f = step == 0 ? L : fp12_mul_by_line_pair(f, L);
    step++;
    if ((BLS_X_ABS >> i) & 1ull) {
      f = fp12_mul_by_line_pair(f, line_mul_line(load(step, 0), load(step, 1)));
      step++;
    }
  }
  return fp12_conj(f);
}

template <int NP>
DI fp12 miller_loop_multi(const g1a (&P)[NP], const g2a (&Q)[NP], const bool (&active)[NP]) {
  g2proj T[NP];
#pragma unroll
  for (int k = 0; k < NP; k++) T[k] = {Q[k].x, Q[k].y, fp2_one()};
  fp12 f = fp12_one();
  bool first = true;
#pragma unroll 1
  for (int i = 62; i >= 0; i--) {
    if (!first) f = fp12_sqr(f);
#pragma unroll
    for (int k = 0; k < NP; k++) {
      fp2 l00, l01, l11;
      miller_dbl_step(T[k], l00, l01, l11, P[k].x, P[k].y);
      if (active[k]) f = fp12_mul_by_014(f, l00, l01, l11);
    }
    first = false;
    if ((BLS_X_ABS >> i) & 1ull) {
#pragma unroll
      for (int k = 0; k < NP; k++) {
        fp2 l00, l01, l11;
        miller_add_step(T[k], Q[k], l00, l01, l11, P[k].x, P[k].y);
        if (active[k]) f = fp12_mul_by_014(f, l00, l01, l11);
      }
    }
  }
  return fp12_conj(f);
}

DI fp12 fexp_easy(const fp12& f) {
  fp12 t = fp12_mul(fp12_conj(f), fp12_inv(f));
  return fp12_mul(fp12_frob2(t), t);
}

template <typename Load>
DI fp12 fp12_pow_x_abs_reload(Load load) {
  constexpr uint64_t NSQ = 1ull | (2ull << 6) | (3ull << 12) | (9ull << 18) | (32ull << 24) | (16ull << 30);
  fp12 r = load();
#pragma unroll 1
  for (int s = 0; s < 6; s++) {
    const int n = (int)((NSQ >> (6 * s)) & 63u);
#pragma unroll 1
    for (int k = 0; k < n; k++) r = fp12_cyclotomic_sqr(r);
    if (s < 5) r = fp12_mul(r, load());
  }
  return r;
}

template <int MODE, typename LX, typename LC, typename LG>
DI fp12 fexp_step(LX lx, LC lc, LG lg) {
  fp12 r = fp12_conj(fp12_pow_x_abs_reload(lx));
  if (MODE == 0 || MODE == 1) return fp12_mul(r, fp12_conj(lx()));
  if (MODE == 2) return fp12_mul(r, fp12_frob(lx()));
  if (MODE == 3) return r;
  r = fp12_mul(r, fp12_frob2(lc()));
  r = fp12_mul(r, fp12_conj(lc()));
  r = fp12_mul(r, fp12_cyclotomic_sqr(lg()));
  return fp12_mul(r, lg());
}

DI fp12 final_exponentiation(const fp12& f) {
  const fp12 g = fexp_easy(f);
  auto none = [&]() { return g; };
  const fp12 a = fexp_step<0>([&]() { return g; }, none, none);
  const fp12 b = fexp_step<1>([&]() { return a; }, none, none);
  const fp12 c = fexp_step<2>([&]() { return b; }, none, none);
  const fp12 t = fexp_step<3>([&]() { return c; }, none, none);
  return fexp_step<4>([&]() { return t; }, [&]() { return c; }, [&]() { return g; });
}

}
```

### drand_amd/csrc/testhooks.cpp

```cpp
#include "../../include/blsverify_testing.h"
#include "host_internal.h"
#include "testops_list.h"

static const bls::TestOpInfo* find_test_op(const char* name, int* op) {
  if (!name) return nullptr;
  const bls::TestOpInfo* tab = bls::test_op_table();
  for (int k = 0; k < bls::TOP_COUNT; k++)
    if (!strcmp(tab[k].name, name)) {
      if (op) *op = k;
      return &tab[k];
    }
  return nullptr;
}

extern "C" {

int blsv_test_lagrange(const uint32_t* idx, size_t t, uint32_t* out) {
  if (!idx || !out) return BLSV_EINVAL;
  for (size_t i = 0; i < t; i++)
    for (size_t j = 0; j < i; j++)
      if (idx[i] == idx[j]) return BLSV_EINVAL;
  host_lagrange(idx, t, out);
  return BLSV_OK;
}

int blsv_test_rlc_seed(blsv_ctx* c, const uint8_t* seed32) {
  if (!c) return BLSV_EINVAL;
  c->rlc.seed_pinned = seed32 != nullptr;
  if (seed32) memcpy(c->rlc.seed, seed32, 32);
  return BLSV_OK;
}

int blsv_test_rlc_sums(blsv_ctx* c, uint64_t first_round, const uint8_t* prev0, size_t prev0_len,
                       const uint8_t* sigs96, size_t n, uint8_t* out_a96, uint8_t* out_b96) {
  if (!c) return BLSV_EINVAL;
  if (!n || !sigs96 || !prev0 || !out_a96 || !out_b96 || (prev0_len != 32 && prev0_len != 96))
    return fail(c, BLSV_EINVAL, "test_rlc_sums: bad arguments");
  (void)hipSetDevice(c->device);
  Tail tail;
  tail.randomized = true;
  int rc = rlc_draw_seed(c, tail.seed);
  if (rc) return rc;
  rc = ensure_workspace(c, n);
  if (rc) return rc;
  blsk::ChainedSrc src;
  rc = stage_chain(c, first_round, prev0, prev0_len, false, sigs96, n, src);
  if (rc) return rc;
  rlc_state& r = c->rlc;
  size_t done = 0;
  rc = for_each_pass(c, n, [&](size_t base, size_t cnt) {
    const size_t ng = blsk::rlc_groups(cnt, r.group);
    int prc = run_head(c, {src.sigs, 96, 0}, base, cnt, tail, c->stream,
                       [&](size_t b, size_t m, hipStream_t st) { hash_chained(c, src, b, m, st); });
    if (prc) return prc;
    prc = rlc_sums(c, base, cnt, tail.seed, c->stream);
    if (prc) return prc;
    HIPCHK(c, r.out96.ensure(2 * ng * 96));
    uint8_t* d_out = r.out96.as<uint8_t>();
    blsk::launch_rlc_compress(r.gH.as<uint32_t>(), r.g_hinf.as<uint8_t>(), ng, d_out, c->stream);
    blsk::launch_rlc_compress(r.gS.as<uint32_t>(), r.g_sinf.as<uint8_t>(), ng, d_out + ng * 96, c->stream);
    HIPCHK(c, hipGetLastError());
    HIPCHK(c, hipMemcpyAsync(out_a96 + done * 96, d_out, ng * 96, hipMemcpyDeviceToHost, c->stream));
    HIPCHK(c, hipMemcpyAsync(out_b96 + done * 96, d_out + ng * 96, ng * 96, hipMemcpyDeviceToHost, c->stream));
    HIPCHK(c, hipStreamSynchronize(c->stream));
    c->io_up_off = 0;
    done += ng;
    return BLSV_OK;
  });
  return rc ? rc : (int)done;
}

int blsv_test_spec_stats(blsv_ctx* c, uint64_t* hits, uint64_t* misses) {
  if (!c || !hits || !misses) return BLSV_EINVAL;
  *hits = c->spec_hits;
  *misses = c->spec_misses;
  return BLSV_OK;
}

int blsv_test_tail_split(blsv_ctx* c, size_t q) {
  if (!c) return BLSV_EINVAL;
  c->tail_q = q == SIZE_MAX ? c->tail_q_dev : q;
  return BLSV_OK;
}

int blsv_test_generic_chains(blsv_ctx* c, int on) {
  if (!c) return BLSV_EINVAL;
  blsk::g_generic_chains_all = on != 0;
  return BLSV_OK;
}

int blsv_lat_trace_enable(blsv_ctx* c, int on) {
  if (!c) return BLSV_EINVAL;
  (void)hipSetDevice(c->device);
  if (blsk::lat_trace_enable(on, c->stream) != 0) return fail(c, BLSV_EHIP, "lat_trace_enable: symbol copy failed");
  return BLSV_OK;
}

int blsv_lat_trace(blsv_ctx* c, uint64_t* ticks, int n, double* ticks_per_us, int clear) {
  if (!c || n < 0 || (n && !ticks)) return BLSV_EINVAL;
  (void)hipSetDevice(c->device);
  HIPCHK(c, hipDeviceSynchronize());
  int got = 0;
  if (n) {
    got = blsk::lat_trace_read(ticks, n, c->stream);
    if (got < 0) return fail(c, BLSV_EHIP, "lat_trace: symbol copy failed");
  }
  if (ticks_per_us) {
    int khz = 0;
    HIPCHK(c, hipDeviceGetAttribute(&khz, hipDeviceAttributeWallClockRate, c->device));
    *ticks_per_us = khz / 1000.0;
  }
  if (clear && blsk::lat_trace_clear(c->stream) != 0) return fail(c, BLSV_EHIP, "lat_trace: clear failed");
  HIPCHK(c, hipStreamSynchronize(c->stream));
  return got;
}

int blsv_test_fp_mul(blsv_ctx* c, const uint32_t* a, const uint32_t* b, size_t n, uint32_t* out) {
  if (!c || (n && (!a || !b || !out))) return BLSV_EINVAL;
  (void)hipSetDevice(c->device);
  DBuf da, db, dout;
  HIPCHK(c, da.ensure(n * 48));
  HIPCHK(c, db.ensure(n * 48));
  HIPCHK(c, dout.ensure(n * 48));
  HIPCHK(c, hipMemcpyAsync(da.p, a, n * 48, hipMemcpyHostToDevice, c->stream));
  HIPCHK(c, hipMemcpyAsync(db.p, b, n * 48, hipMemcpyHostToDevice, c->stream));
  blsk::launch_test_fp_mul(da.as<uint32_t>(), db.as<uint32_t>(), n, dout.as<uint32_t>(), c->stream);
  HIPCHK(c, hipGetLastError());
  HIPCHK(c, hipMemcpyAsync(out, dout.p, n * 48, hipMemcpyDeviceToHost, c->stream));
  HIPCHK(c, hipStreamSynchronize(c->stream));
  return BLSV_OK;
}

int blsv_test_pairing(blsv_ctx* c, const uint32_t* p, const uint32_t* q, size_t n, uint32_t* out_f) {
  if (!c || (n && (!p || !q || !out_f))) return BLSV_EINVAL;
  (void)hipSetDevice(c->device);
  DBuf dp, dq, dout;
  HIPCHK(c, dp.ensure(n * 96));
  HIPCHK(c, dq.ensure(n * 192));
  HIPCHK(c, dout.ensure(n * 576));
  HIPCHK(c, hipMemcpyAsync(dp.p, p, n * 96, hipMemcpyHostToDevice, c->stream));
  HIPCHK(c, hipMemcpyAsync(dq.p, q, n * 192, hipMemcpyHostToDevice, c->stream));
  blsk::launch_test_pairing(dp.as<uint32_t>(), dq.as<uint32_t>(), n, dout.as<uint32_t>(), c->stream);
  HIPCHK(c, hipGetLastError());
  HIPCHK(c, hipMemcpyAsync(out_f, dout.p, n * 576, hipMemcpyDeviceToHost, c->stream));
  HIPCHK(c, hipStreamSynchronize(c->stream));
  return BLSV_OK;
}

int blsv_test_final_exp(blsv_ctx* c, const uint32_t* f, size_t n, uint32_t* out_pipeline, uint32_t* out_ref) {
  if (!c || (n && (!f || !out_pipeline || !out_ref))) return BLSV_EINVAL;
  if (n > kMaxChunk) return BLSV_EINVAL;
  (void)hipSetDevice(c->device);
  int rc = ensure_workspace(c, n);
  if (rc) return rc;
  if (n > c->cap) return fail(c, BLSV_EINVAL, "test_final_exp: more than the context chunk");
  if (!n) return BLSV_OK;
  DBuf din, dout, dref;
  HIPCHK(c, din.ensure(n * 576));
  HIPCHK(c, dout.ensure(n * 576));
  HIPCHK(c, dref.ensure(n * 576));
  const Staging w = staging(c);
  HIPCHK(c, hipMemcpyAsync(din.p, f, n * 576, hipMemcpyHostToDevice, c->stream));
  HIPCHK(c, hipMemsetAsync(w.cls, 0, n, c->stream));
  blsk::launch_test_pack_fp12(din.as<uint32_t>(), n, w.F, c->stream);
  blsk::launch_test_final_exp_ref(w.F, n, dref.as<uint32_t>(), c->stream);
  const size_t mn = tail_split_main(n, c->tail_q);
  final_exp(c, n, 0, mn, w.cls, c->stream, dout.as<uint32_t>());
  final_exp(c, n, mn, n - mn, w.cls, c->stream, dout.as<uint32_t>());
  blsk::launch_test_unpack_fp12(dout.as<uint32_t>(), n, din.as<uint32_t>(), c->stream);
  HIPCHK(c, hipMemcpyAsync(out_pipeline, din.p, n * 576, hipMemcpyDeviceToHost, c->stream));
  blsk::launch_test_unpack_fp12(dref.as<uint32_t>(), n, dout.as<uint32_t>(), c->stream);
  HIPCHK(c, hipMemcpyAsync(out_ref, dout.p, n * 576, hipMemcpyDeviceToHost, c->stream));
  HIPCHK(c, hipGetLastError());
  HIPCHK(c, hipStreamSynchronize(c->stream));
  return BLSV_OK;
}

int blsv_test_op_info(int index, const char** name, int* in_fp, int* out_fp, int* lanes) {
  if (index < 0 || index >= bls::TOP_COUNT) return BLSV_EINVAL;
  const bls::TestOpInfo& t = bls::test_op_table()[index];
  if (name) *name = t.name;
  if (in_fp) *in_fp = t.nin;
  if (out_fp) *out_fp = t.nout;
  if (lanes) *lanes = t.kind == 3 ? 3 : 1;
  return BLSV_OK;
}

int blsv_test_op(blsv_ctx* c, const char* name, const uint32_t* in, size_t n, uint32_t* out) {
  int op = 0;
  const bls::TestOpInfo* t = find_test_op(name, &op);
  if (!c || !t || (n && (!in || !out))) return BLSV_EINVAL;
  if (n > kMaxChunk) return BLSV_EINVAL;
  if (!n) return BLSV_OK;
  (void)hipSetDevice(c->device);
  const size_t in_bytes = n * (size_t)t->nin * 48, out_bytes = n * (size_t)t->nout * 48;
  DBuf din, dout, dpark;
  HIPCHK(c, din.ensure(in_bytes));
  HIPCHK(c, dout.ensure(out_bytes));
  if (t->kind == 3) HIPCHK(c, dpark.ensure(blsk::TRI_PARK_WORDS(n) * 4));
  HIPCHK(c, hipMemcpyAsync(din.p, in, in_bytes, hipMemcpyHostToDevice, c->stream));
  HIPCHK(c, hipMemsetAsync(dout.p, 0xA5, out_bytes, c->stream));
  const bool ran = t->kind == 2
                       ? blsk::launch_test_op_mf(op, din.as<uint32_t>(), n, dout.as<uint32_t>(), c->stream)
                       : blsk::launch_test_op(op, din.as<uint32_t>(), n, dout.as<uint32_t>(),
                                              t->kind == 3 ? dpark.as<uint32_t>() : nullptr, c->stream);
  if (!ran) return fail(c, BLSV_EINVAL, "test_op: no kernel for this op");
  HIPCHK(c, hipGetLastError());
  HIPCHK(c, hipMemcpyAsync(out, dout.p, out_bytes, hipMemcpyDeviceToHost, c->stream));
  HIPCHK(c, hipStreamSynchronize(c->stream));
  return BLSV_OK;
}

int blsv_test_hash_to_g2(blsv_ctx* c, const uint8_t* msgs, const uint32_t* msg_lens, size_t n, uint32_t* out,
                         uint8_t* inf) {
  if (!c || (n && (!msg_lens || !out || !inf))) return BLSV_EINVAL;
  if (n > kMaxChunk) return BLSV_EINVAL;
  (void)hipSetDevice(c->device);
  int rc = ensure_workspace(c, n);
  if (rc) return rc;
  if (n > c->cap) return fail(c, BLSV_EINVAL, "test_hash_to_g2: more than the context chunk");
  rc = upload_messages(c, msgs, msg_lens, n);
  if (rc) return rc;
  DBuf dout;
  HIPCHK(c, dout.ensure(n * 192));
  hash_uploaded(c, 0, n, c->stream);
  blsk::launch_test_unpack_g2(c->H.as<uint32_t>(), n, dout.as<uint32_t>(), c->stream);
  HIPCHK(c, hipGetLastError());
  HIPCHK(c, hipMemcpyAsync(out, dout.p, n * 192, hipMemcpyDeviceToHost, c->stream));
  HIPCHK(c, hipMemcpyAsync(inf, c->h_inf.p, n, hipMemcpyDeviceToHost, c->stream));
  HIPCHK(c, hipStreamSynchronize(c->stream));
  return BLSV_OK;
}

}
```

### drand_amd/csrc/tlock.cpp

```cpp
#include "host_internal.h"

static int tlock_prepare_sig(blsv_ctx* c, const uint8_t* sig96, hipStream_t st, uint8_t* sig_class) {
  tlock_state& t = c->tlock;
  if (!t.valid || memcmp(t.sig, sig96, 96) != 0) {
    t.valid = false;
    HIPCHK(c, t.d_sig.ensure(96));
    HIPCHK(c, t.S.ensure(blsk::S_WORDS * 4));
    HIPCHK(c, t.s_inf.ensure(1));
    HIPCHK(c, t.s_cls.ensure(1));
    HIPCHK(c, t.tab.ensure(blsk::kTlockTabWords * 4));
    HIPCHK(c, hipMemcpyAsync(t.d_sig.p, sig96, 96, hipMemcpyHostToDevice, st));
    {
      StageTimer tm(c, ST_TLOCK, 1, st);
      blsk::launch_decompress_g2(t.d_sig.as<uint8_t>(), 96, 0, 0, 1, t.S.as<uint32_t>(), t.s_inf.as<uint8_t>(),
                                 t.s_cls.as<uint8_t>(), st);
      blsk::launch_tlock_prepare(t.S.as<uint32_t>(), t.s_inf.as<uint8_t>(), t.s_cls.as<uint8_t>(),
                                 t.tab.as<uint32_t>(), st);
    }
    HIPCHK(c, hipGetLastError());
    uint8_t cls = 0xff;
    HIPCHK(c, hipMemcpyAsync(&cls, t.s_cls.p, 1, hipMemcpyDeviceToHost, st));
    HIPCHK(c, hipStreamSynchronize(st));
    memcpy(t.sig, sig96, 96);
    t.cls = cls;
    t.valid = true;
    if (cls == BLSV_REJ_OK) t.prepared++;
  }
  if (sig_class) *sig_class = t.cls;
  if (t.cls != BLSV_REJ_OK) return fail(c, BLSV_EINVAL, "tlock_open: signature rejected (class %d)", (int)t.cls);
  return BLSV_OK;
}

static int tlock_pass(blsv_ctx* c, const uint8_t* d_us, size_t cnt, uint8_t* d_out, uint8_t* d_cls_out,
                      hipStream_t st) {
  const tlock_state& t = c->tlock;
  const Staging w = staging(c);
  uint32_t* U = w.H;
  uint8_t* u_inf = w.h_inf;
  uint8_t* ucls = w.s_inf;
  {
    StageTimer tm(c, ST_DECOMP, cnt, st);
    blsk::launch_decompress_g1(d_us, cnt, U, u_inf, ucls, st);
  }
  HIPCHK(c, hipMemcpyAsync(w.cls, ucls, cnt, hipMemcpyDeviceToDevice, st));
  {
    StageTimer tm(c, ST_TLOCK, cnt, st);
    blsk::launch_tlock_f(t.tab.as<uint32_t>(), U, u_inf, ucls, t.s_inf.as<uint8_t>(), cnt, w.F, st);
  }
  {
    StageTimer tm(c, ST_FEXP, cnt, st);
    blsk::launch_final_exp(w.F, w.FW, cnt, 0, cnt, w.cls, st, w.LN, w.HQ);
  }
  blsk::launch_tlock_encode(w.HQ, ucls, cnt, d_out, st);
  if (d_cls_out) HIPCHK(c, hipMemcpyAsync(d_cls_out, ucls, cnt, hipMemcpyDeviceToDevice, st));
  HIPCHK(c, hipGetLastError());
  return BLSV_OK;
}

static int tlock_passes(blsv_ctx* c, bool host, const uint8_t* us, size_t n, uint8_t* out, uint8_t* cls,
                        hipStream_t st) {
  int rc = ensure_workspace(c, n);
  if (rc) return rc;
  for (size_t base = 0; base < n; base += c->cap) {
    const size_t cnt = std::min(c->cap, n - base);
    const uint8_t* pass_us = us + base * BLSV_U_LEN;
    uint8_t* pass_out = out + base * BLSV_GT_LEN;
    if (host) {
      HIPCHK(c, h2d(c, c->S.p, pass_us, cnt * BLSV_U_LEN));
      rc = tlock_pass(c, c->S.as<uint8_t>(), cnt, c->F.as<uint8_t>(), nullptr, st);
      if (rc) return rc;
      HIPCHK(c, download_sync(c, {{pass_out, c->F.p, cnt * BLSV_GT_LEN}, {cls + base, c->s_inf.p, cnt}}));
    } else {
      rc = tlock_pass(c, pass_us, cnt, pass_out, cls ? cls + base : nullptr, st);
      if (rc) return rc;
    }
  }
  c->tlock.items += n;
  return BLSV_OK;
}

extern "C" {

int blsv_tlock_open(blsv_ctx* c, const uint8_t* sig96, const uint8_t* us48, size_t n, uint8_t* out_gt576, uint8_t* ok,
                    uint8_t* reject_class, uint8_t* sig_class) {
  if (!c) return BLSV_EINVAL;
  if (!sig96 || (n && (!us48 || !out_gt576 || !ok))) return fail(c, BLSV_EINVAL, "tlock_open: bad arguments");
  (void)hipSetDevice(c->device);
  int rc = tlock_prepare_sig(c, sig96, c->stream, sig_class);
  if (rc) return rc;
  if (!n) return BLSV_OK;
  std::vector<uint8_t> own;
  uint8_t* cls = reject_class;
  if (!cls) {
    own.resize(n);
    cls = own.data();
  }
  rc = tlock_passes(c, true, us48, n, out_gt576, cls, c->stream);
  if (rc) return rc;
  for (size_t i = 0; i < n; i++) ok[i] = cls[i] == BLSV_REJ_OK;
  return BLSV_OK;
}

int blsv_tlock_open_dev(blsv_ctx* c, const uint8_t* sig96, const uint8_t* d_us48, size_t n, uint8_t* d_out_gt576,
                        uint8_t* d_reject_class, void* stream) {
  if (!c) return BLSV_EINVAL;
  if (!sig96 || (n && (!d_us48 || !d_out_gt576)) || ((uintptr_t)d_out_gt576 & 3))
    return fail(c, BLSV_EINVAL, "tlock_open_dev: bad arguments");
  (void)hipSetDevice(c->device);
  hipStream_t st = stream ? (hipStream_t)stream : c->stream;
  int rc = tlock_prepare_sig(c, sig96, st, nullptr);
  if (rc) return rc;
  if (!n) return BLSV_OK;
  return tlock_passes(c, false, d_us48, n, d_out_gt576, d_reject_class, st);
}

int blsv_tlock_stats(blsv_ctx* c, uint64_t* prepared, uint64_t* items) {
  if (!c) return BLSV_EINVAL;
  if (prepared) *prepared = c->tlock.prepared;
  if (items) *items = c->tlock.items;
  return BLSV_OK;
}

}
```

### drand_amd/csrc/tower.h

```cpp
#pragma once
#include "fp.h"

namespace bls {

struct fp2 {
  fp c0, c1;
};
struct fp6 {
  fp2 c0, c1, c2;
};
struct fp12 {
  fp6 c0, c1;
};

DI fp2 fp2_load_const(const uint32_t (&c)[2][12]) { return {fp_load_const(c[0]), fp_load_const(c[1])}; }
DI fp2 fp2_zero() { return {fp_zero(), fp_zero()}; }
DI fp2 fp2_one() { return {fp_one(), fp_zero()}; }
DI bool fp2_is_zero(const fp2& a) { return fp_is_zero(a.c0) & fp_is_zero(a.c1); }
DI bool fp2_eq(const fp2& a, const fp2& b) { return fp_eq(a.c0, b.c0) & fp_eq(a.c1, b.c1); }
DI fp2 fp2_select(bool c, const fp2& a, const fp2& b) { return {fp_select(c, a.c0, b.c0), fp_select(c, a.c1, b.c1)}; }
DI fp2 fp2_add(const fp2& a, const fp2& b) {
  uint32_t s0[12], d0[12], s1[12], d1[12];
  unsigned c0 = 0, b0 = 0, c1 = 0, b1 = 0;
#pragma unroll
// ... 93 lines not shown
#pragma unroll
      for (int c = 0; c < N; c++) d[c][i] = __builtin_subc(P2_RAW[i], x[c].l[i], b[c], &b[c]);
#pragma unroll
    for (int i = 0; i < 12; i++)
#pragma unroll
      for (int c = 0; c < N; c++) y[c][i] = sub[c] ? d[c][i] : x[c].l[i];
  }
  uint32_t t[N][12];
  unsigned h[N];
  {
    uint32_t w[N][12];
    unsigned cs[N], cw[N];
#pragma unroll
    for (int c = 0; c < N; c++) cs[c] = cw[c] = h[c] = 0;
#pragma unroll
    for (int i = 0; i < 12; i++)
#pragma unroll
      for (int c = 0; c < N; c++) {
        const uint32_t si = __builtin_addc(u[c].l[i], y[c][i], cs[c], &cs[c]);
        w[c][i] = __builtin_addc(si, si, cw[c], &cw[c]);
      }
#pragma unroll
    for (int i = 0; i < 12; i++)
#pragma unroll
      for (int c = 0; c < N; c++) t[c][i] = __builtin_addc(w[c][i], u[c].l[i], h[c], &h[c]);
  }
  u12 qp[N];
#pragma unroll
  for (int c = 0; c < N; c++) qp[c] = kp(fp_quot_top(t[c], h[c]));
  unsigned b[N];
#pragma unroll
  for (int c = 0; c < N; c++) b[c] = 0;
#pragma unroll
  for (int i = 0; i < 12; i++)
#pragma unroll
    for (int c = 0; c < N; c++) r[c].l[i] = __builtin_subc(t[c][i], qp[c][i], b[c], &b[c]);
}
template <typename KP = KpMad>
DI fp2 fp2_3u_pm_2x(const fp2& u, const fp2& x, bool sub, KP kp = KP()) {
  const fp uu[2] = {u.c0, u.c1}, xx[2] = {x.c0, x.c1};
  const bool ss[2] = {sub, sub};
  fp r[2];
  fp_3u_pm_2x_n<2>(uu, xx, ss, r, kp);
  return {r[0], r[1]};
}

DI fp2 fp2_neg(const fp2& a) {
  uint32_t d0[12], d1[12];
  unsigned b0 = 0, b1 = 0;
#pragma unroll
  for (int i = 0; i < 12; i++) {
    d0[i] = __builtin_subc(P2_RAW[i], a.c0.l[i], b0, &b0);
    d1[i] = __builtin_subc(P2_RAW[i], a.c1.l[i], b1, &b1);
  }
  const uint32_t m0 = fp_raw_is_zero(a.c0) ? 0u : 0xffffffffu, m1 = fp_raw_is_zero(a.c1) ? 0u : 0xffffffffu;
  fp2 r;
#pragma unroll
  for (int i = 0; i < 12; i++) {
    r.c0.l[i] = d0[i] & m0;
    r.c1.l[i] = d1[i] & m1;
  }
  return r;
}
DI fp2 fp2_conj(const fp2& a) { return {a.c0, fp_neg(a.c1)}; }

DI u24 fp2_to_u24(const fp2& a) { return u24_of(fp_to_u12(a.c0), fp_to_u12(a.c1)); }
DI fp2 fp2_from_u24(const u24& v) { return {fp_from_u12(u24_lo(v)), fp_from_u12(u24_hi(v))}; }

DI fp2 fp2_mul(const fp2& a, const fp2& b) {
  fp2_arg_store(fp2_to_u24(b));
  return fp2_from_u24(fp2_mul_u24(fp2_to_u24(a)));
}
DI fp2 fp2_sqr(const fp2& a) { return fp2_from_u24(fp2_sqr_u24(fp2_to_u24(a))); }
template <bool KARA>
DI fp2 fp2_mul_inl_t(const fp2& a, const fp2& b) {
  BLS_COUNT_MUL();
  BLS_COUNT_MUL();
  BLS_COUNT_MUL();
  return fp2_from_u24(fp2_mul_body_t<KARA>(fp2_to_u24(a), fp_to_u12(b.c0), fp_to_u12(b.c1)));
}
DI fp2 fp2_mul_inl(const fp2& a, const fp2& b) { return fp2_mul_inl_t<BLS_FP2_KARA_INL>(a, b); }
#ifndef BLS_LINES_KARA
#define BLS_LINES_KARA 3
#endif
template <int SITE>
DI fp2 fp2_mul_inl_k(const fp2& a, const fp2& b) { return fp2_mul_inl_t<((BLS_LINES_KARA >> SITE) & 1) != 0>(a, b); }
DI fp2 fp2_sqr_inl(const fp2& a) {
  BLS_COUNT_MUL();
  BLS_COUNT_MUL();
  return fp2_from_u24(fp2_sqr_body(fp2_to_u24(a)));
}

DI fp2 fp2_mul_fp(const fp2& a, const fp& b) { return {fp_mul(a.c0, b), fp_mul(a.c1, b)}; }
DI fp2 fp2_mul_fp_inl(const fp2& a, const fp& b) {
  const fp c0 = fp_mul_inl(a.c0, b);
  BLS_SCHED_FENCE();
  return {c0, fp_mul_inl(a.c1, b)};
}
DI fp2 fp2_mul3(const fp2& a) { return {fp_mul3(a.c0), fp_mul3(a.c1)}; }

DI fp2 fp2_mul_xi(const fp2& a) {
  uint32_t d[12], e[12], s[12], u[12];
  unsigned bd = 0, ce = 0, cs = 0, bu = 0;
#pragma unroll
  for (int i = 0; i < 12; i++) {
    d[i] = __builtin_subc(a.c0.l[i], a.c1.l[i], bd, &bd);
    s[i] = __builtin_addc(a.c0.l[i], a.c1.l[i], cs, &cs);
    e[i] = __builtin_addc(d[i], P2_RAW[i], ce, &ce);
    u[i] = __builtin_subc(s[i], P2_RAW[i], bu, &bu);
  }
  fp2 r;
#pragma unroll
  for (int i = 0; i < 12; i++) {
    r.c0.l[i] = bd ? e[i] : d[i];
    r.c1.l[i] = bu ? s[i] : u[i];
  }
  return r;
}

DI fp2 fp2_inv(const fp2& a) {
  fp n = fp_add(fp_sqr(a.c0), fp_sqr(a.c1));
  fp ni = fp_inv(n);
  return {fp_mul(a.c0, ni), fp_neg(fp_mul(a.c1, ni))};
}

DI bool fp2_sgn0(const fp2& a) {
  fp r0 = fp_from_mont(a.c0);
  fp r1 = fp_from_mont(a.c1);
  bool s0 = r0.l[0] & 1u;
  bool z0 = fp_is_zero(r0);
  bool s1 = r1.l[0] & 1u;
  return s0 | (z0 & s1);
}

DI bool fp2_lex_largest(const fp2& a) {
  fp r1 = fp_from_mont(a.c1);
  if (!fp_is_zero(r1)) return fp_raw_gt_half(r1);
  return fp_raw_gt_half(fp_from_mont(a.c0));
}

DI fp2 fp2_sqrt_with_norm_root(const fp2& a, const fp& s) {
  fp ap = fp_half(fp_add(a.c0, s));
  fp am = fp_half(fp_sub(a.c0, s));
  ap = fp_select(fp_is_zero(ap), am, ap);
  fp w = fp_pow_sqrt_inv(ap);
  fp t = fp_mul(w, ap);
  bool direct = fp_eq(fp_sqr(t), ap);
  fp inv2t = fp_half(fp_select(direct, w, fp_neg(w)));
  fp other = fp_mul(a.c1, inv2t);
  return {fp_select(direct, t, other), fp_select(direct, other, t)};
}

DI fp fp2_norm(const fp2& a) { return fp_add(fp_sqr(a.c0), fp_sqr(a.c1)); }

DI fp fp_norm_root(const fp& n, bool& is_sq) {
  fp s = fp_mul(fp_pow_sqrt_inv(n), n);
  is_sq = fp_eq(fp_sqr(s), n);
  return s;
}

DI bool fp2_sqrt(fp2& out, const fp2& a) {
  bool ok;
  fp s = fp_norm_root(fp2_norm(a), ok);
  fp2 r = fp2_sqrt_with_norm_root(a, s);
  ok = ok & fp2_eq(fp2_sqr(r), a);
  out = r;
  return ok;
}

DI fp2 fp2_half(const fp2& a) { return {fp_half(a.c0), fp_half(a.c1)}; }

DI fp6 fp6_zero() { return {fp2_zero(), fp2_zero(), fp2_zero()}; }
DI fp6 fp6_one() { return {fp2_one(), fp2_zero(), fp2_zero()}; }
DI fp6 fp6_add(const fp6& a, const fp6& b) { return {fp2_add(a.c0, b.c0), fp2_add(a.c1, b.c1), fp2_add(a.c2, b.c2)}; }
DI fp6 fp6_sub(const fp6& a, const fp6& b) { return {fp2_sub(a.c0, b.c0), fp2_sub(a.c1, b.c1), fp2_sub(a.c2, b.c2)}; }
DI fp6 fp6_neg(const fp6& a) { return {fp2_neg(a.c0), fp2_neg(a.c1), fp2_neg(a.c2)}; }
DI bool fp6_eq(const fp6& a, const fp6& b) { return fp2_eq(a.c0, b.c0) & fp2_eq(a.c1, b.c1) & fp2_eq(a.c2, b.c2); }

DI fp6 fp6_mul_v(const fp6& a) { return {fp2_mul_xi(a.c2), a.c0, a.c1}; }

#ifndef BLS_F6_LIN
#define BLS_F6_LIN 1
#endif
struct Words12 {
  uint32_t w[12];
};
constexpr Words12 kp_words(uint32_t k) {
  Words12 r{};
  uint64_t c = 0;
  for (int i = 0; i < 12; i++) {
    c = (uint64_t)k * P_RAW[i] + (c >> 32);
    r.w[i] = (uint32_t)c;
  }
  return r;
}
#ifndef BLS_HOST
template <int K>
DI uint32_t* kp_lds_tab() {
  static __shared__ __attribute__((aligned(16))) uint32_t tab[K * 12];
  return tab;
}
template <int K>
DI void kp_lds_init() {
  uint32_t* tab = kp_lds_tab<K>();
  for (unsigned j = threadIdx.x; j < (unsigned)K * 12u; j += blockDim.x) {
    const uint32_t k = j / 12u, word = j % 12u;
    uint64_t c = 0;
    uint32_t w = 0;
#pragma unroll
    for (int i = 0; i < 12; i++) {
      c = (uint64_t)k * P_RAW[i] + (c >> 32);
      if ((uint32_t)i == word) w = (uint32_t)c;
    }
    tab[j] = w;
  }
  __syncthreads();
}
template <int K>
struct KpLdsK {
  DI u12 operator()(uint32_t q) const {
    q = q < (uint32_t)(K - 1) ? q : (uint32_t)(K - 1);
    const uint4* r = reinterpret_cast<const uint4*>(kp_lds_tab<K>()) + 3u * q;
    const uint4 a = r[0], b = r[1], c = r[2];
    u12 w;
    w[0] = a.x, w[1] = a.y, w[2] = a.z, w[3] = a.w, w[4] = b.x, w[5] = b.y;
    w[6] = b.z, w[7] = b.w, w[8] = c.x, w[9] = c.y, w[10] = c.z, w[11] = c.w;
    return w;
  }
};
#endif

template <typename KP>
DI fp2 fp2_lin_reduce(const uint32_t (&t0)[12], unsigned h0, const uint32_t (&t1)[12], unsigned h1, KP kp) {
  const u12 w0 = kp(fp_quot_top(t0, h0)), w1 = kp(fp_quot_top(t1, h1));
  fp2 r;
  unsigned b0 = 0, b1 = 0;
#pragma unroll
  for (int i = 0; i < 12; i++) {
    r.c0.l[i] = __builtin_subc(t0[i], w0[i], b0, &b0);
    r.c1.l[i] = __builtin_subc(t1[i], w1[i], b1, &b1);
  }
  return r;
}
template <typename KP>
DI fp2 kara6_c0(const fp2& m12, const fp2& t0, const fp2& t1, const fp2& t2, KP kp) {
  constexpr Words12 B0 = kp_words(6), B1 = kp_words(8);
  uint32_t pa0[12], pa1[12], na0[12], na1[12];
  {
    unsigned cu0 = 0, cu1 = 0, c0 = 0, c1 = 0, c2 = 0, c3 = 0;
#pragma unroll
    for (int i = 0; i < 12; i++) {
      const uint32_t u0 = __builtin_addc(t1.c0.l[i], t2.c0.l[i], cu0, &cu0);
      const uint32_t u1 = __builtin_addc(t1.c1.l[i], t2.c1.l[i], cu1, &cu1);
      pa0[i] = __builtin_addc(m12.c0.l[i], u1, c0, &c0);
      pa1[i] = __builtin_addc(m12.c0.l[i], m12.c1.l[i], c1, &c1);
      na0[i] = __builtin_addc(m12.c1.l[i], u0, c2, &c2);
      na1[i] = __builtin_addc(u0, u1, c3, &c3);
    }
  }
  uint32_t T0[12], T1[12];
  unsigned h0 = 0, h1 = 0;
  {
    unsigned c0 = 0, c1 = 0, b0 = 0, b1 = 0;
#pragma unroll
    for (int i = 0; i < 12; i++) {
      const uint32_t p0 = __builtin_addc(pa0[i], t0.c0.l[i], c0, &c0);
      const uint32_t p1 = __builtin_addc(pa1[i], t0.c1.l[i], c1, &c1);
      const uint32_t n0 = __builtin_subc(B0.w[i], na0[i], b0, &b0);
      const uint32_t n1 = __builtin_subc(B1.w[i], na1[i], b1, &b1);
      T0[i] = __builtin_addc(p0, n0, h0, &h0);
      T1[i] = __builtin_addc(p1, n1, h1, &h1);
    }
  }
  return fp2_lin_reduce(T0, h0, T1, h1, kp);
}
template <typename KP>
DI fp2 kara6_c1(const fp2& m01, const fp2& t0, const fp2& t1, const fp2& t2, KP kp) {
  constexpr Words12 B0 = kp_words(6), B1 = kp_words(4);
  uint32_t pa0[12], pa1[12], na0[12], na1[12];
  {
    unsigned c0 = 0, c1 = 0, c2 = 0, c3 = 0;
#pragma unroll
    for (int i = 0; i < 12; i++) {
      pa0[i] = __builtin_addc(m01.c0.l[i], t2.c0.l[i], c0, &c0);
      pa1[i] = __builtin_addc(m01.c1.l[i], t2.c0.l[i], c1, &c1);
      na0[i] = __builtin_addc(t0.c0.l[i], t1.c0.l[i], c2, &c2);
      na1[i] = __builtin_addc(t0.c1.l[i], t1.c1.l[i], c3, &c3);
    }
  }
  uint32_t T0[12], T1[12];
  unsigned h0 = 0, h1 = 0;
  {
    unsigned c1 = 0, c2 = 0, b0 = 0, b1 = 0;
#pragma unroll
    for (int i = 0; i < 12; i++) {
      const uint32_t p1 = __builtin_addc(pa1[i], t2.c1.l[i], c1, &c1);
      const uint32_t m0 = __builtin_addc(na0[i], t2.c1.l[i], c2, &c2);
      const uint32_t n0 = __builtin_subc(B0.w[i], m0, b0, &b0);
      const uint32_t n1 = __builtin_subc(B1.w[i], na1[i], b1, &b1);
      T0[i] = __builtin_addc(pa0[i], n0, h0, &h0);
      T1[i] = __builtin_addc(p1, n1, h1, &h1);
    }
  }
  return fp2_lin_reduce(T0, h0, T1, h1, kp);
}
template <typename KP>
// ... 1 lines not shown
  constexpr Words12 B = kp_words(4);
  uint32_t T0[12], T1[12];
  unsigned h0 = 0, h1 = 0;
  {
    unsigned c0 = 0, c1 = 0, c2 = 0, c3 = 0, b0 = 0, b1 = 0;
#pragma unroll
    for (int i = 0; i < 12; i++) {
      const uint32_t p0 = __builtin_addc(m02.c0.l[i], t1.c0.l[i], c0, &c0);
      const uint32_t p1 = __builtin_addc(m02.c1.l[i], t1.c1.l[i], c1, &c1);
      const uint32_t s0 = __builtin_addc(t0.c0.l[i], t2.c0.l[i], c2, &c2);
      const uint32_t s1 = __builtin_addc(t0.c1.l[i], t2.c1.l[i], c3, &c3);
      const uint32_t n0 = __builtin_subc(B.w[i], s0, b0, &b0);
      const uint32_t n1 = __builtin_subc(B.w[i], s1, b1, &b1);
      T0[i] = __builtin_addc(p0, n0, h0, &h0);
      T1[i] = __builtin_addc(p1, n1, h1, &h1);
    }
  }
  return fp2_lin_reduce(T0, h0, T1, h1, kp);
}

template <typename LB, typename KP>
DI fp6 fp6_mul_lin_lb(const fp6& a, LB lb, KP kp) {
  const fp2 t0 = fp2_mul(a.c0, lb(0));
  const fp2 t1 = fp2_mul(a.c1, lb(1));
  const fp2 t2 = fp2_mul(a.c2, lb(2));
  const fp2 c0 = kara6_c0(fp2_mul(fp2_add_lazy(a.c1, a.c2), fp2_add_lazy(lb(1), lb(2))), t0, t1, t2, kp);
  const fp2 c1 = kara6_c1(fp2_mul(fp2_add_lazy(a.c0, a.c1), fp2_add_lazy(lb(0), lb(1))), t0, t1, t2, kp);
  const fp2 c2 = kara6_c2(fp2_mul(fp2_add_lazy(a.c0, a.c2), fp2_add_lazy(lb(0), lb(2))), t0, t1, t2, kp);
  return {c0, c1, c2};
}
template <typename KP = KpMad>
DI fp6 fp6_mul_lin(const fp6& a, const fp6& b, KP kp = KP()) {
  return fp6_mul_lin_lb(a, [&](int c) { return c == 0 ? b.c0 : (c == 1 ? b.c1 : b.c2); }, kp);
}

DI fp6 fp6_mul(const fp6& a, const fp6& b) {
  fp2 t0 = fp2_mul(a.c0, b.c0);
  fp2 t1 = fp2_mul(a.c1, b.c1);
  fp2 t2 = fp2_mul(a.c2, b.c2);
  fp2 c0 = fp2_add(fp2_mul_xi(fp2_sub(fp2_sub(fp2_mul(fp2_add_lazy(a.c1, a.c2), fp2_add_lazy(b.c1, b.c2)), t1), t2)), t0);
  fp2 c1 = fp2_add(fp2_sub(fp2_sub(fp2_mul(fp2_add_lazy(a.c0, a.c1), fp2_add_lazy(b.c0, b.c1)), t0), t1), fp2_mul_xi(t2));
  fp2 c2 = fp2_add(fp2_sub(fp2_sub(fp2_mul(fp2_add_lazy(a.c0, a.c2), fp2_add_lazy(b.c0, b.c2)), t0), t2), t1);
  return {c0, c1, c2};
}

DI fp6 fp6_add_lazy(const fp6& a, const fp6& b) {
  return {fp2_add_lazy(a.c0, b.c0), fp2_add_lazy(a.c1, b.c1), fp2_add_lazy(a.c2, b.c2)};
}

DI fp6 fp6_sqr(const fp6& a) {
  fp2 s0 = fp2_sqr(a.c0);
  fp2 ab = fp2_mul(a.c0, a.c1);
  fp2 s1 = fp2_dbl(ab);
  fp2 s2 = fp2_sqr(fp2_add_lazy(fp2_sub(a.c0, a.c1), a.c2));
  fp2 bc = fp2_mul(a.c1, a.c2);
  fp2 s3 = fp2_dbl(bc);
  fp2 s4 = fp2_sqr(a.c2);
  fp2 c0 = fp2_add(fp2_mul_xi(s3), s0);
  fp2 c1 = fp2_add(fp2_mul_xi(s4), s1);
  fp2 c2 = fp2_sub(fp2_sub(fp2_add(fp2_add(s1, s2), s3), s0), s4);
  return {c0, c1, c2};
}

DI fp6 fp6_mul_by_01(const fp6& a, const fp2& b0, const fp2& b1) {
  fp2 t0 = fp2_mul(a.c0, b0);
  fp2 t1 = fp2_mul(a.c1, b1);
  fp2 c0 = fp2_add(fp2_mul_xi(fp2_sub(fp2_mul(fp2_add_lazy(a.c1, a.c2), b1), t1)), t0);
  fp2 c1 = fp2_sub(fp2_sub(fp2_mul(fp2_add_lazy(a.c0, a.c1), fp2_add_lazy(b0, b1)), t0), t1);
  fp2 c2 = fp2_add(fp2_sub(fp2_mul(fp2_add_lazy(a.c0, a.c2), b0), t0), t1);
  return {c0, c1, c2};
}

DI fp6 fp6_mul_by_1(const fp6& a, const fp2& b1) {
  return {fp2_mul_xi(fp2_mul(a.c2, b1)), fp2_mul(a.c0, b1), fp2_mul(a.c1, b1)};
}

DI fp6 fp6_inv(const fp6& a) {
  fp2 t0 = fp2_sub(fp2_sqr(a.c0), fp2_mul_xi(fp2_mul(a.c1, a.c2)));
  fp2 t1 = fp2_sub(fp2_mul_xi(fp2_sqr(a.c2)), fp2_mul(a.c0, a.c1));
  fp2 t2 = fp2_sub(fp2_sqr(a.c1), fp2_mul(a.c0, a.c2));
  fp2 d = fp2_add(fp2_mul(a.c0, t0), fp2_mul_xi(fp2_add(fp2_mul(a.c2, t1), fp2_mul(a.c1, t2))));
  fp2 di = fp2_inv(d);
  return {fp2_mul(t0, di), fp2_mul(t1, di), fp2_mul(t2, di)};
}

DI fp12 fp12_one() { return {fp6_one(), fp6_zero()}; }
DI bool fp12_eq(const fp12& a, const fp12& b) { return fp6_eq(a.c0, b.c0) & fp6_eq(a.c1, b.c1); }
DI bool fp12_is_one(const fp12& a) { return fp12_eq(a, fp12_one()); }
DI fp12 fp12_conj(const fp12& a) { return {a.c0, fp6_neg(a.c1)}; }

DI fp12 fp12_mul(const fp12& a, const fp12& b) {
  fp6 t0 = fp6_mul(a.c0, b.c0);
  fp6 t1 = fp6_mul(a.c1, b.c1);
  fp6 c1 = fp6_sub(fp6_sub(fp6_mul(fp6_add_lazy(a.c0, a.c1), fp6_add_lazy(b.c0, b.c1)), t0), t1);
  fp6 c0 = fp6_add(t0, fp6_mul_v(t1));
  return {c0, c1};
}

template <typename KP>
DI fp12 fp12_sqr_lin(const fp12& a, KP kp) {
  fp6 ab = fp6_mul_lin(a.c0, a.c1, kp);
  fp6 t = fp6_mul_lin(fp6_add_lazy(a.c0, a.c1), fp6_add_lazy(a.c0, fp6_mul_v(a.c1)), kp);
  fp6 c0 = fp6_sub(fp6_sub(t, ab), fp6_mul_v(ab));
  fp6 c1 = fp6_add(ab, ab);
  return {c0, c1};
}

DI fp12 fp12_sqr(const fp12& a) {
  fp6 ab = fp6_mul(a.c0, a.c1);
  fp6 t = fp6_mul(fp6_add_lazy(a.c0, a.c1), fp6_add_lazy(a.c0, fp6_mul_v(a.c1)));
  fp6 c0 = fp6_sub(fp6_sub(t, ab), fp6_mul_v(ab));
  fp6 c1 = fp6_add(ab, ab);
  return {c0, c1};
}

DI fp12 fp12_mul_by_014(const fp12& f, const fp2& l00, const fp2& l01, const fp2& l11) {
  fp6 a = fp6_mul_by_01(f.c0, l00, l01);
  fp6 b = fp6_mul_by_1(f.c1, l11);
  fp6 c = fp6_mul_by_01(fp6_add_lazy(f.c0, f.c1), l00, fp2_add_lazy(l01, l11));
  fp6 c1 = fp6_sub(fp6_sub(c, a), b);
  fp6 c0 = fp6_add(a, fp6_mul_v(b));
  return {c0, c1};
}

DI void fp4_sqr(fp2& c0, fp2& c1, const fp2& a, const fp2& b) {
  fp2 t0 = fp2_sqr(a);
  fp2 t1 = fp2_sqr(b);
  c0 = fp2_add(fp2_mul_xi(t1), t0);
  c1 = fp2_sub(fp2_sub(fp2_sqr(fp2_add_lazy(a, b)), t0), t1);
}

DI fp12 fp12_cyclotomic_sqr(const fp12& f) {
  fp2 z0 = f.c0.c0, z4 = f.c0.c1, z3 = f.c0.c2, z2 = f.c1.c0, z1 = f.c1.c1, z5 = f.c1.c2;
  fp2 t0, t1, t2, t3;
  fp4_sqr(t0, t1, z0, z1);
  z0 = fp2_add(fp2_dbl(fp2_sub(t0, z0)), t0);
  z1 = fp2_add(fp2_dbl(fp2_add(t1, z1)), t1);
  fp4_sqr(t0, t1, z2, z3);
  fp4_sqr(t2, t3, z4, z5);
  z4 = fp2_add(fp2_dbl(fp2_sub(t0, z4)), t0);
  z5 = fp2_add(fp2_dbl(fp2_add(t1, z5)), t1);
  t0 = fp2_mul_xi(t3);
  z2 = fp2_add(fp2_dbl(fp2_add(t0, z2)), t0);
  z3 = fp2_add(fp2_dbl(fp2_sub(t2, z3)), t2);
  return {{z0, z4, z3}, {z2, z1, z5}};
}

DI fp12 fp12_inv(const fp12& a) {
  fp6 d = fp6_sub(fp6_sqr(a.c0), fp6_mul_v(fp6_sqr(a.c1)));
  fp6 di = fp6_inv(d);
  return {fp6_mul(a.c0, di), fp6_neg(fp6_mul(a.c1, di))};
}

DI fp12 fp12_frob(const fp12& a) {
  fp12 r;
  r.c0.c0 = fp2_conj(a.c0.c0);
  r.c1.c0 = fp2_mul(fp2_conj(a.c1.c0), fp2_load_const(FROB1_GAMMA[1]));
  r.c0.c1 = fp2_mul(fp2_conj(a.c0.c1), fp2_load_const(FROB1_GAMMA[2]));
  r.c1.c1 = fp2_mul(fp2_conj(a.c1.c1), fp2_load_const(FROB1_GAMMA[3]));
  r.c0.c2 = fp2_mul(fp2_conj(a.c0.c2), fp2_load_const(FROB1_GAMMA[4]));
  r.c1.c2 = fp2_mul(fp2_conj(a.c1.c2), fp2_load_const(FROB1_GAMMA[5]));
  return r;
}

DI fp12 fp12_frob2(const fp12& a) {
  fp12 r;
  r.c0.c0 = a.c0.c0;
  r.c1.c0 = fp2_mul_fp(a.c1.c0, fp_load_const(FROB2_GAMMA[1][0]));
  r.c0.c1 = fp2_mul_fp(a.c0.c1, fp_load_const(FROB2_GAMMA[2][0]));
  r.c1.c1 = fp2_mul_fp(a.c1.c1, fp_load_const(FROB2_GAMMA[3][0]));
  r.c0.c2 = fp2_mul_fp(a.c0.c2, fp_load_const(FROB2_GAMMA[4][0]));
  r.c1.c2 = fp2_mul_fp(a.c1.c2, fp_load_const(FROB2_GAMMA[5][0]));
  return r;
}

}
```

### drand_amd/csrc/verify.cpp

```cpp
#include <sys/random.h>

#include <thread>

#include "host_internal.h"

static bool serial_stages() {
  static const bool on = [] {
    const char* e = getenv("BLSV_SERIAL_STAGES");
    return e && e[0] == '1';
  }();
  return on;
}

static void head_decompress(blsv_ctx* c, const SigSrc& sig, size_t base, size_t cnt, const Tail& tail, hipStream_t st) {
  const Staging w = staging(c);
  if (tail.fused_subgroup() && !blsk::g_generic_chains_all)
    blsk::launch_decompress_g2_only(sig.d, sig.stride, sig.offset, base, cnt, w.S, w.s_inf, w.cls, st);
  else
    blsk::launch_decompress_g2(sig.d, sig.stride, sig.offset, base, cnt, w.S, w.s_inf, w.cls, st);
}

int run_head(blsv_ctx* c, const SigSrc& sig, size_t base, size_t cnt, const Tail& tail, hipStream_t st,
             const HashFn& hash) {
  if (serial_stages()) {
// ... 235 lines not shown
      cls = own.data();
    }
    HIPCHK(c, download_sync(c, {{cls, c->cls.p, n}}));
    put_first_bad(fold_classes(cls, n, ok_bitmap));
    return BLSV_OK;
  }
  Tail tail;
  tail.randomized = randomized;
  if (randomized && (rc = rlc_draw_seed(c, tail.seed))) return rc;
  PassOut out;
  rc = ctx_outputs(c, n, reject_class != nullptr, out);
  if (rc) return rc;
  rc = run_passes(c, n, sig, pk, hash, tail, out, c->stream);
  if (rc) return rc;
  const size_t words = (n + 63) / 64;
  std::vector<uint64_t> w(words + 1, 0);
  uint64_t fb = UINT64_MAX;
  HIPCHK(c, download_sync(c, {{w.data(), c->bitmap.p, words * 8},
                              {&fb, c->first_bad.p, 8},
                              {reject_class, c->misc.p, reject_class ? n : 0}}));
  if (ok_bitmap) bitmap_words_to_bytes(w.data(), n, ok_bitmap);
  put_first_bad(fb);
  return BLSV_OK;
}

int decode_g1(blsv_ctx* c, const uint8_t* pk48, size_t cnt, DBuf& tab, DBuf& inf, std::vector<uint8_t>& cls) {
  HIPCHK(c, tab.ensure(cnt * blsk::G1_WORDS * 4));
  HIPCHK(c, inf.ensure(cnt));
  HIPCHK(c, c->g1_cls.ensure(cnt));
  HIPCHK(c, c->misc.ensure(cnt * 48));
  HIPCHK(c, hipMemcpyAsync(c->misc.p, pk48, cnt * 48, hipMemcpyHostToDevice, c->stream));
  blsk::launch_decompress_g1(c->misc.as<uint8_t>(), cnt, tab.as<uint32_t>(), inf.as<uint8_t>(),
                             c->g1_cls.as<uint8_t>(), c->stream);
  HIPCHK(c, hipGetLastError());
  cls.assign(cnt, 0);
  HIPCHK(c, hipMemcpyAsync(cls.data(), c->g1_cls.p, cnt, hipMemcpyDeviceToHost, c->stream));
  HIPCHK(c, hipStreamSynchronize(c->stream));
  return BLSV_OK;
}

int upload_messages(blsv_ctx* c, const uint8_t* msgs, const uint32_t* msg_lens, size_t n) {
  std::vector<uint64_t> off(n + 1, 0);
  for (size_t i = 0; i < n; i++) off[i + 1] = off[i] + msg_lens[i];
  if (off[n] && !msgs) return fail(c, BLSV_EINVAL, "messages: %llu message bytes but no buffer",
                                   (unsigned long long)off[n]);
  HIPCHK(c, c->in_msgs.ensure(off[n] + 1));
  HIPCHK(c, c->in_off.ensure((n + 1) * 8));
  HIPCHK(c, c->in_len.ensure(n * 4 + 4));
  const size_t staged_max = kIoCap / 4;
  HIPCHK(c, h2d(c, c->in_msgs.p, msgs, off[n]));
  HIPCHK(c, h2d(c, c->in_off.p, off.data(), (n + 1) * 8));
  HIPCHK(c, h2d(c, c->in_len.p, msg_lens, n * 4));
  if ((n + 1) * 8 > staged_max) HIPCHK(c, hipStreamSynchronize(c->stream));
  return BLSV_OK;
}

int svc_verify_mixed(blsv_ctx* c, size_t n, const uint8_t* msgs, const uint64_t* off, const uint32_t* lens,
                     const uint8_t* sigs96, const uint32_t* idx, const uint32_t* d_tab, const uint8_t* d_tab_inf,
                     uint8_t* cls_out) {
  if (!n) return BLSV_OK;
  if (n > kMaxChunk) return fail(c, BLSV_EINVAL, "service batch larger than %zu", kMaxChunk);
  (void)hipSetDevice(c->device);
  int rc = ensure_workspace(c, std::min(n, c->chunk));
  if (rc) return rc;
  const size_t mbytes = off[n];
  const SvcLayout l = svc_layout(n, mbytes);
  HIPCHK(c, c->pin.ensure(std::max(l.total, n + 8)));
  uint8_t* h = c->pin.as<uint8_t>();
  memcpy(h, off, (n + 1) * 8);
  memcpy(h + l.o_len, lens, n * 4);
  memcpy(h + l.o_idx, idx, n * 4);
  memcpy(h + l.o_sig, sigs96, n * 96);
  if (mbytes) memcpy(h + l.o_msg, msgs, mbytes);
  HIPCHK(c, c->arena.ensure(l.total));
  HIPCHK(c, c->misc.ensure(n + 64));
  HIPCHK(c, hipMemcpyAsync(c->arena.p, h, l.total, hipMemcpyHostToDevice, c->stream));
  uint8_t* d = c->arena.as<uint8_t>();
  const uint64_t* d_off = reinterpret_cast<const uint64_t*>(d);
  const uint32_t* d_len = reinterpret_cast<const uint32_t*>(d + l.o_len);
  const uint8_t* d_msg = d + l.o_msg;
  const SigSrc sig{d + l.o_sig, 96, 0};
  const PkSel pk{d_tab, d_tab_inf, reinterpret_cast<const uint32_t*>(d + l.o_idx)};
  if (use_lat(c, n)) {
    blsk::launch_lat_messages(d_msg, d_off, d_len, sig.d, 96, 0, n, pk.tab, pk.inf, pk.idx, c->misc.as<uint8_t>(),
                              nullptr, nullptr, c->stream);
  } else {
    PassOut out;
    rc = ctx_outputs(c, n, true, out);
    if (rc) return rc;
    rc = run_passes(
        c, n, sig, pk,
        [&](size_t base, size_t cnt, hipStream_t st) { hash_messages(c, d_msg, d_off, d_len, base, cnt, st); }, Tail(),
        out, c->stream);
    if (rc) return rc;
  }
  HIPCHK(c, hipGetLastError());
  HIPCHK(c, hipMemcpyAsync(h, c->misc.p, n, hipMemcpyDeviceToHost, c->stream));
  HIPCHK(c, hipStreamSynchronize(c->stream));
  memcpy(cls_out, h, n);
  return BLSV_OK;
}

int stage_chain(blsv_ctx* c, uint64_t first_round, const uint8_t* prevs, size_t prev0_len, bool prev_rows,
                const uint8_t* sigs96, size_t n, blsk::ChainedSrc& src) {
  HIPCHK(c, c->in_sigs.ensure(n * 96 + 96));
  HIPCHK(c, c->seeds.ensure(prev_rows ? n * 96 + 96 : 96));
  if (n) {
    HIPCHK(c, h2d(c, c->in_sigs.p, sigs96, n * 96));
    HIPCHK(c, h2d(c, c->seeds.p, prevs, prev_rows ? n * 96 : prev0_len));
  }
  src = {c->in_sigs.as<uint8_t>(), c->seeds.as<uint8_t>(), first_round, prev_rows ? 1 : std::max<uint64_t>(n, 1),
         (uint32_t)prev0_len};
  return BLSV_OK;
}

static int chained_host(blsv_ctx* c, const char* name, bool prev_rows, bool randomized, uint64_t first_round,
                        const uint8_t* prevs, size_t prev0_len, const uint8_t* sigs96, size_t n, uint8_t* ok_bitmap,
                        uint64_t* first_bad, uint8_t* reject_class) {
  if (!c->has_group) return fail(c, BLSV_ENOGROUP, "%s: no group key set", name);
  if (n && (!sigs96 || !prevs || (prev0_len != 32 && prev0_len != 96)))
    return fail(c, BLSV_EINVAL, "%s: %s must be 32 or 96 bytes", name, prev_rows ? "row 0's prev" : "prev0");
  if (n > SIZE_MAX / 96 - 1) return fail(c, BLSV_EINVAL, "%s: %zu rounds overflow the byte count", name, n);
  (void)hipSetDevice(c->device);
  blsk::ChainedSrc src;
  const int rc = stage_chain(c, first_round, prevs, prev0_len, prev_rows, sigs96, n, src);
  if (rc) return rc;
  const PkSel pk = group_pk(c);
  return verify_host(
      c, n, {src.sigs, 96, 0}, pk, [&](size_t base, size_t cnt, hipStream_t st) { hash_chained(c, src, base, cnt, st); },
      [&](uint8_t* cls) { blsk::launch_lat_chained(src, 0, n, pk.tab, pk.inf, cls, c->stream); }, randomized,
      first_round, nullptr, ok_bitmap, first_bad, reject_class);
}

static int unchained_host(blsv_ctx* c, const char* name, bool randomized, const uint64_t* rounds, uint64_t first_round,
                          const uint8_t* sigs96, size_t n, uint8_t* ok_bitmap, uint64_t* first_bad,
                          uint8_t* reject_class) {
  if (!c->has_group) return fail(c, BLSV_ENOGROUP, "%s: no group key set", name);
  if (n && !sigs96) return fail(c, BLSV_EINVAL, "%s: null signatures", name);
  (void)hipSetDevice(c->device);
  HIPCHK(c, c->in_sigs.ensure(n * 96 + 96));
  if (n) HIPCHK(c, h2d(c, c->in_sigs.p, sigs96, n * 96));
  const uint64_t* d_rounds = nullptr;
  if (rounds && n) {
    HIPCHK(c, c->in_rounds.ensure(n * 8));
    HIPCHK(c, h2d(c, c->in_rounds.p, rounds, n * 8));
    d_rounds = c->in_rounds.as<uint64_t>();
  }
  const PkSel pk = group_pk(c);
  const SigSrc sig{c->in_sigs.as<uint8_t>(), 96, 0};
  return verify_host(
      c, n, sig, pk,
      [&](size_t base, size_t cnt, hipStream_t st) {
        const Staging w = staging(c);
        blsk::launch_hash_unchained(d_rounds, first_round, base, cnt, w.H, w.h_inf, w.HQ, st);
      },
      [&](uint8_t* cls) { blsk::launch_lat_unchained(d_rounds, first_round, sig.d, 0, n, pk.tab, pk.inf, cls, c->stream); },
      randomized, first_round, rounds, ok_bitmap, first_bad, reject_class);
}

static int run_lat(blsv_ctx* c, size_t n, const LatFn& lat, const PassOut& out, hipStream_t st) {
  {
    StageTimer tm(c, ST_LAT, n, st);
    lat(c->cls.as<uint8_t>());
  }
  blsk::launch_finish(c->cls.as<uint8_t>(), 0, n, out.bitmap, out.first_bad, out.label0, st);
  if (out.cls) HIPCHK(c, hipMemcpyAsync(out.cls, c->cls.p, n, hipMemcpyDeviceToDevice, st));
  HIPCHK(c, hipGetLastError());
  return BLSV_OK;
}

static int chained_dev(blsv_ctx* c, const char* name, bool randomized, uint64_t first_round, uint64_t seg_len,
                       uint64_t seg_phase, const uint8_t* d_seeds96, size_t seed0_len, const uint8_t* d_sigs96, size_t n,
                       uint64_t* d_bitmap, uint64_t* d_first_bad, uint8_t* d_reject_class, void* stream) {
  if (!c->has_group) return fail(c, BLSV_ENOGROUP, "%s: no group key set", name);
  if (n && (!d_seeds96 || !d_sigs96 || !d_bitmap || !d_first_bad || (seed0_len != 32 && seed0_len != 96)))
    return fail(c, BLSV_EINVAL, "%s: bad arguments", name);
  if (seg_phase && (!seg_len || seg_phase >= seg_len))
    return fail(c, BLSV_EINVAL, "%s: seg_phase must be < seg_len", name);
  (void)hipSetDevice(c->device);
  hipStream_t st = stream ? (hipStream_t)stream : c->stream;
  Tail tail;
  tail.randomized = randomized;
  int rc = randomized ? rlc_draw_seed(c, tail.seed) : BLSV_OK;
  if (rc) return rc;
  HIPCHK(c, hipMemsetAsync(d_first_bad, 0xff, 8, st));
  rc = ensure_workspace(c, n);
  if (rc) return rc;
  const blsk::ChainedSrc src{d_sigs96,           d_seeds96, first_round, seg_len ? seg_len : std::max<uint64_t>(n, 1),
                             (uint32_t)seed0_len, seg_phase};
  const PkSel pk = group_pk(c);
  const PassOut out{d_bitmap, (unsigned long long*)d_first_bad, d_reject_class, first_round};
  if (use_lat(c, n))
    return run_lat(c, n, [&](uint8_t* cls) { blsk::launch_lat_chained(src, 0, n, pk.tab, pk.inf, cls, st); }, out, st);
  return run_passes(
      c, n, {d_sigs96, 96, 0}, pk, [&](size_t base, size_t cnt, hipStream_t s) { hash_chained(c, src, base, cnt, s); },
      tail, out, st);
}

extern "C" {

int blsv_verify_chained(blsv_ctx* c, uint64_t first_round, const uint8_t* prev0, size_t prev0_len,
                        const uint8_t* sigs96, size_t n, uint8_t* ok_bitmap, uint64_t* first_bad,
                        uint8_t* reject_class) {
  if (!c) return BLSV_EINVAL;
  return chained_host(c, "verify_chained", false, false, first_round, prev0, prev0_len, sigs96, n, ok_bitmap, first_bad,
                      reject_class);
}

int blsv_verify_prevs(blsv_ctx* c, uint64_t first_round, const uint8_t* prevs96, size_t prev0_len,
                      const uint8_t* sigs96, size_t n, uint8_t* ok_bitmap, uint64_t* first_bad,
                      uint8_t* reject_class) {
  if (!c) return BLSV_EINVAL;
  return chained_host(c, "verify_prevs", true, false, first_round, prevs96, prev0_len, sigs96, n, ok_bitmap, first_bad,
                      reject_class);
}

int blsv_verify_chained_rlc(blsv_ctx* c, uint64_t first_round, const uint8_t* prev0, size_t prev0_len,
                            const uint8_t* sigs96, size_t n, uint8_t* ok_bitmap, uint64_t* first_bad,
                            uint8_t* reject_class) {
  if (!c) return BLSV_EINVAL;
  const bool rlc = use_rlc(c, n);
  return chained_host(c, rlc ? "verify_chained_rlc" : "verify_chained", false, rlc, first_round, prev0, prev0_len,
                      sigs96, n, ok_bitmap, first_bad, reject_class);
}

int blsv_verify_unchained(blsv_ctx* c, const uint64_t* rounds, uint64_t first_round, const uint8_t* sigs96, size_t n,
                          uint8_t* ok_bitmap, uint64_t* first_bad, uint8_t* reject_class) {
  if (!c) return BLSV_EINVAL;
  return unchained_host(c, "verify_unchained", false, rounds, first_round, sigs96, n, ok_bitmap, first_bad,
                        reject_class);
}

int blsv_verify_unchained_rlc(blsv_ctx* c, const uint64_t* rounds, uint64_t first_round, const uint8_t* sigs96,
                              size_t n, uint8_t* ok_bitmap, uint64_t* first_bad, uint8_t* reject_class) {
  if (!c) return BLSV_EINVAL;
  const bool rlc = use_rlc(c, n);
  return unchained_host(c, rlc ? "verify_unchained_rlc" : "verify_unchained", rlc, rounds, first_round, sigs96, n,
                        ok_bitmap, first_bad, reject_class);
}

int blsv_verify_chained_dev(blsv_ctx* c, uint64_t first_round, uint64_t seg_len, uint64_t seg_phase,
                            const uint8_t* d_seeds96, size_t seed0_len, const uint8_t* d_sigs96, size_t n,
                            uint64_t* d_bitmap, uint64_t* d_first_bad, uint8_t* d_reject_class, void* stream) {
  if (!c) return BLSV_EINVAL;
  return chained_dev(c, "verify_chained_dev", false, first_round, seg_len, seg_phase, d_seeds96, seed0_len, d_sigs96, n,
                     d_bitmap, d_first_bad, d_reject_class, stream);
}

int blsv_verify_chained_rlc_dev(blsv_ctx* c, uint64_t first_round, uint64_t seg_len, uint64_t seg_phase,
                                const uint8_t* d_seeds96, size_t seed0_len, const uint8_t* d_sigs96, size_t n,
                                uint64_t* d_bitmap, uint64_t* d_first_bad, uint8_t* d_reject_class, void* stream) {
  if (!c) return BLSV_EINVAL;
  const bool rlc = use_rlc(c, n);
  return chained_dev(c, rlc ? "verify_chained_rlc_dev" : "verify_chained_dev", rlc, first_round, seg_len, seg_phase,
                     d_seeds96, seed0_len, d_sigs96, n, d_bitmap, d_first_bad, d_reject_class, stream);
}

int blsv_verify_chained_multi(blsv_ctx* const* ctxs, size_t n_ctx, const size_t* shard_counts, uint64_t first_round,
                              const uint8_t* prev0, size_t prev0_len, const uint8_t* sigs96, size_t n,
                              uint8_t* ok_bitmap, uint64_t* first_bad, uint8_t* reject_class) {
  if (!ctxs || n_ctx == 0) return BLSV_EINVAL;
  for (size_t k = 0; k < n_ctx; k++) {
    if (!ctxs[k]) return BLSV_EINVAL;
    for (size_t j = 0; j < k; j++)
      if (ctxs[j] == ctxs[k]) return fail(ctxs[k], BLSV_EINVAL, "verify_chained_multi: context %zu repeated", k);
  }
  blsv_ctx* c0 = ctxs[0];
  for (size_t k = 0; k < n_ctx; k++) {
    if (!ctxs[k]->has_group) return fail(ctxs[k], BLSV_ENOGROUP, "verify_chained_multi: context %zu has no group", k);
    if (ctxs[k]->group_bytes != c0->group_bytes)
      return fail(ctxs[k], BLSV_EINVAL, "verify_chained_multi: context %zu holds another group", k);
  }
  if (n && (!sigs96 || !prev0 || (prev0_len != 32 && prev0_len != 96)))
    return fail(c0, BLSV_EINVAL, "verify_chained_multi: prev0 must be 32 or 96 bytes");
  std::vector<size_t> cnt(n_ctx), start(n_ctx);
  size_t sum = 0;
  for (size_t k = 0; k < n_ctx; k++) {
    cnt[k] = shard_counts ? shard_counts[k] : n / n_ctx + (k < n % n_ctx ? 1 : 0);
    start[k] = sum;
    sum += cnt[k];
  }
  if (sum != n) return fail(c0, BLSV_EINVAL, "verify_chained_multi: shard counts sum to %zu, not %zu", sum, n);
  std::vector<std::vector<uint8_t>> bms(n_ctx);
  std::vector<uint64_t> fbs(n_ctx, UINT64_MAX);
  std::vector<int> rcs(n_ctx, BLSV_OK);
  auto shard = [&](size_t k) {
    if (!cnt[k]) return;
    bms[k].assign((cnt[k] + 7) / 8, 0);
    const bool head = start[k] == 0;
    const uint8_t* halo = head ? prev0 : sigs96 + (start[k] - 1) * 96;
    rcs[k] = blsv_verify_chained(ctxs[k], first_round + start[k], halo, head ? prev0_len : 96, sigs96 + start[k] * 96,
                                 cnt[k], bms[k].data(), &fbs[k], reject_class ? reject_class + start[k] : nullptr);
  };
  std::vector<std::thread> th;
  for (size_t k = 1; k < n_ctx; k++)
    if (cnt[k]) th.emplace_back(shard, k);
  shard(0);
  for (auto& t : th) t.join();
  for (size_t k = 0; k < n_ctx; k++)
    if (rcs[k]) return rcs[k];
  uint64_t fb = UINT64_MAX;
  for (size_t k = 0; k < n_ctx; k++) fb = std::min(fb, fbs[k]);
  if (first_bad) *first_bad = fb;
  if (ok_bitmap && n) {
    memset(ok_bitmap, 0, (n + 7) / 8);
    for (size_t k = 0; k < n_ctx; k++)
      if (cnt[k]) or_bits_at(ok_bitmap, bms[k].data(), cnt[k], start[k]);
// ... 74 lines not shown
```

### drand_amd/engine.py

```python
from __future__ import annotations

import ctypes
from dataclasses import dataclass

from . import _lib
from ._lib import u8p, u32p, u64p


class EngineError(RuntimeError):
    def __init__(self, code, msg):
        super().__init__(f"blsverify error {code}: {msg}")
        self.code = code


@dataclass
class BatchResult:
    ok: list
    first_bad: int | None
    reject_class: list

    @property
    def all_ok(self):
        return self.first_bad is None

# ... 311 lines not shown
        self._check(self.lib.blsv_test_rlc_seed(self._h, _lib.buf(seed32) if seed32 is not None else None))

    def test_rlc_sums(self, first_round, prev0, sigs):
        n = len(sigs)
        sigb = b"".join(bytes(s) for s in sigs)
        cap = -(-n // 8) + n // 16384 + 1
        a, b = _lib.out_buf(cap * 96), _lib.out_buf(cap * 96)
        ng = self.lib.blsv_test_rlc_sums(self._h, first_round, _lib.buf(prev0), len(prev0), _lib.buf(sigb), n, a, b)
        if ng < 0:
            raise EngineError(ng, self.lib.blsv_last_error(self._h).decode())
        ab, bb = bytes(a), bytes(b)
        return ([ab[96 * k:96 * k + 96] for k in range(ng)], [bb[96 * k:96 * k + 96] for k in range(ng)])

    def tlock_open(self, sig, us):
        sig = bytes(sig)
        us = [bytes(u) for u in us]
        if len(sig) != 96:
            raise ValueError("the round signature is 96 bytes")
        if any(len(u) != 48 for u in us):
            raise ValueError("U values must be 48 bytes (reject wrong lengths host-side)")
        n = len(us)
        out = _lib.out_buf(n * 576)
        ok = _lib.out_buf(n)
        cls = _lib.out_buf(n)
        sc = ctypes.c_uint8()
        rc = self.lib.blsv_tlock_open(self._h, _lib.buf(sig), _lib.buf(b"".join(us)), n, out, ok, cls,
                                      ctypes.cast(ctypes.byref(sc), u8p))
        if rc == _lib.BLSV_EINVAL and sc.value:
            raise SignatureRejected(rc, self.lib.blsv_last_error(self._h).decode(), sc.value)
        self._check(rc)
        ob = bytes(out)
        oks = [bool(x) for x in list(ok)[:n]]
        return TlockResult(oks, list(cls)[:n], [ob[576 * i:576 * i + 576] if oks[i] else None for i in range(n)])

    def tlock_open_dev(self, sig, d_us, n, d_out, d_cls=None, stream=None):
        sig = bytes(sig)
        if len(sig) != 96:
            raise ValueError("the round signature is 96 bytes")
        self._check(self.lib.blsv_tlock_open_dev(self._h, _lib.buf(sig), d_us, n, d_out, d_cls, stream))

    def tlock_stats(self):
        a, b = ctypes.c_uint64(), ctypes.c_uint64()
        self._check(self.lib.blsv_tlock_stats(self._h, ctypes.byref(a), ctypes.byref(b)))
        return a.value, b.value

    @staticmethod
    def _seal_key(pk48):
        if pk48 is None:
            return None
        pk48 = bytes(pk48)
        if len(pk48) != 48:
            raise ValueError("the public key is 48 bytes")
        return _lib.buf(pk48)

    def tlock_seal(self, round_, scalars, pk48=None):
        sc = [_scalar32(k) for k in scalars]
        n = len(sc)
        us, gt, ok = _lib.out_buf(n * 48), _lib.out_buf(n * 576), _lib.out_buf(n)
        self._check(self.lib.blsv_tlock_seal(self._h, self._seal_key(pk48), int(round_), _lib.buf(b"".join(sc)), n, us,
                                             gt, ok))
        ub, gb = bytes(us), bytes(gt)
        oks = [bool(x) for x in list(ok)[:n]]
        return TsealResult(oks, [ub[48 * i:48 * i + 48] if oks[i] else None for i in range(n)],
                           [gb[576 * i:576 * i + 576] if oks[i] else None for i in range(n)])

    def tlock_seal_dev(self, round_, d_scalars, n, d_us, d_gt, d_ok, pk48=None, stream=None):
        self._check(self.lib.blsv_tlock_seal_dev(self._h, self._seal_key(pk48), int(round_), d_scalars, n, d_us, d_gt,
                                                 d_ok, stream))

    def tlock_seal_stats(self):
        a, b = ctypes.c_uint64(), ctypes.c_uint64()
        self._check(self.lib.blsv_tlock_seal_stats(self._h, ctypes.byref(a), ctypes.byref(b)))
        return a.value, b.value

    STAGES = ("hash", "decompress", "miller", "final_exp", "finish", "lat", "rlc", "tlock")

    def profile(self, on=True):
        self._check(self.lib.blsv_profile_enable(self._h, 1 if on else 0))

    def profile_read(self):
        n = len(self.STAGES)
        ms = (ctypes.c_double * n)()
        la = (ctypes.c_uint64 * n)()
        it = (ctypes.c_uint64 * n)()
        rc = self.lib.blsv_profile_read(self._h, ms, la, it, n)
        if rc < 0:
            raise EngineError(rc, self.lib.blsv_last_error(self._h).decode())
        return {s: (ms[k], la[k], it[k]) for k, s in enumerate(self.STAGES)}

    LAT_MARKS = ("start", "hash", "sig_decoded", "sig_miller", "phase_a", "key_miller", "miller_product",
                 "final_exp", "pow1_start", "pow1_end", "xmd_done", "sswu_done", "iso_add_done", "cofactor_done",
                 "sig_sqrt_done", "sig_subgroup_done")

    def lat_trace_enable(self, on=True):
        self._check(self.lib.blsv_lat_trace_enable(self._h, 1 if on else 0))

    def lat_trace(self, clear=True):
        n = len(self.LAT_MARKS)
        t = (ctypes.c_uint64 * n)()
        rate = ctypes.c_double()
        got = self.lib.blsv_lat_trace(self._h, t, n, ctypes.byref(rate), 1 if clear else 0)
        if got < 0:
            raise EngineError(got, self.lib.blsv_last_error(self._h).decode())
        t0 = t[0]
        return {k: (t[i] - t0) / rate.value for i, k in enumerate(self.LAT_MARKS[:got]) if t[i] and t0}

    def set_lat_max(self, n):
        return self.lib.blsv_set_lat_max(self._h, int(n))

    def set_chunk(self, items):
        return self.lib.blsv_set_chunk(self._h, int(items))

    def workspace_bytes(self):
        return self.lib.blsv_workspace_bytes(self._h)

    def test_fp_mul(self, a_limbs, b_limbs):
        n = len(a_limbs) // 12
        A = (ctypes.c_uint32 * max(len(a_limbs), 1))(*a_limbs)
        B = (ctypes.c_uint32 * max(len(b_limbs), 1))(*b_limbs)
        O = (ctypes.c_uint32 * max(n * 12, 1))()
        self._check(self.lib.blsv_test_fp_mul(self._h, A, B, n, O))
        return list(O)[:n * 12]

    def test_ops(self):
        ops, k = {}, 0
        name, a, b, c = ctypes.c_char_p(), ctypes.c_int(), ctypes.c_int(), ctypes.c_int()
        while self.lib.blsv_test_op_info(k, ctypes.byref(name), ctypes.byref(a), ctypes.byref(b), ctypes.byref(c)) == 0:
            ops[name.value.decode()] = (a.value, b.value, c.value)
            k += 1
        return ops

    def test_op(self, name, operands):
        if self._ops is None:
            self._ops = self.test_ops()
        nin, nout, _ = self._ops[name]
        if len(operands) % nin:
            raise ValueError(f"{name} takes {nin} Fp elements per item")
        n = len(operands) // nin
        raw = b"".join(int(v).to_bytes(48, "little") for v in operands)
        A = (ctypes.c_uint32 * max(len(raw) // 4, 1)).from_buffer_copy(raw if raw else bytes(4))
        O = (ctypes.c_uint32 * max(n * nout * 12, 1))()
        self._check(self.lib.blsv_test_op(self._h, name.encode(), A, n, O))
        ob = bytes(O)
        return [int.from_bytes(ob[48 * k:48 * k + 48], "little") for k in range(n * nout)]

    def test_pairing(self, p_words, q_words):
        n = len(p_words) // 24
        Pp = (ctypes.c_uint32 * max(len(p_words), 1))(*p_words)
        Q = (ctypes.c_uint32 * max(len(q_words), 1))(*q_words)
        O = (ctypes.c_uint32 * max(n * 144, 1))()
        self._check(self.lib.blsv_test_pairing(self._h, Pp, Q, n, O))
        return list(O)[:n * 144]

    def test_final_exp(self, f_words):
        n = len(f_words) // 144
        Fw = (ctypes.c_uint32 * max(len(f_words), 1))(*f_words)
        A = (ctypes.c_uint32 * max(n * 144, 1))()
        B = (ctypes.c_uint32 * max(n * 144, 1))()
        self._check(self.lib.blsv_test_final_exp(self._h, Fw, n, A, B))
        return list(A)[:n * 144], list(B)[:n * 144]

    def test_tail_split(self, q):
        self._check(self.lib.blsv_test_tail_split(self._h, ctypes.c_size_t(-1).value if q is None else int(q)))

    def test_hash_to_g2(self, msgs):
        n = len(msgs)
        lens = (ctypes.c_uint32 * max(n, 1))(*[len(m) for m in msgs])
        O = (ctypes.c_uint32 * max(n * 48, 1))()
        inf = _lib.out_buf(n)
        self._check(self.lib.blsv_test_hash_to_g2(self._h, _lib.buf(b"".join(bytes(m) for m in msgs)), lens, n, O,
                                                  inf))
        return list(O)[:n * 48], list(inf)[:n]

    def spec_stats(self):
        h, m = ctypes.c_uint64(), ctypes.c_uint64()
        self._check(self.lib.blsv_test_spec_stats(self._h, ctypes.byref(h), ctypes.byref(m)))
        return h.value, m.value

    def test_generic_chains(self, on=True):
        self._check(self.lib.blsv_test_generic_chains(self._h, 1 if on else 0))


def verify_chained_multi(engines, first_round, prev0, sigs, counts=None):
    if not engines:
        raise ValueError("verify_chained_multi needs at least one engine")
    lib = engines[0].lib
    n = len(sigs)
    if any(len(s) != 96 for s in sigs):
        raise ValueError("chained signatures must be 96 bytes (reject wrong lengths host-side)")
    sigb = b"".join(bytes(s) for s in sigs)
    hs = (ctypes.c_void_p * len(engines))(*[e._h.value for e in engines])
    cs = None if counts is None else (ctypes.c_size_t * len(engines))(*counts)
    bm = _lib.out_buf((n + 7) // 8)
    fb = ctypes.c_uint64()
    cls = _lib.out_buf(n)
    rc = lib.blsv_verify_chained_multi(hs, len(engines), cs, first_round, _lib.buf(prev0), len(prev0), _lib.buf(sigb),
                                       n, bm, ctypes.byref(fb), cls)
    if rc != 0:
        msgs = "; ".join(lib.blsv_last_error(e._h).decode(errors="replace") for e in engines)
        raise EngineError(rc, f"blsv_verify_chained_multi failed: {msgs}")
    return BatchResult(_bits(bm, n), None if fb.value == 2 ** 64 - 1 else fb.value, list(cls)[:n])


class Service:

    def __init__(self, device: int = 0, gap_us: int = 0, max_wait_us: int = 0, init_torch: bool = True):
        if init_torch:
            try:
                import torch
            except ImportError:
                torch = None
            if torch is not None:
                torch.cuda.set_device(int(device))
                torch.zeros(1, device=torch.device("cuda", int(device)))
        self.lib = _lib.load()
        h = ctypes.c_void_p()
        rc = self.lib.blsv_service_create(int(device), int(gap_us), int(max_wait_us), ctypes.byref(h))
        if rc != 0:
            raise EngineError(rc, f"blsv_service_create(device={device}) failed")
        self._h = h

    def close(self):
        if getattr(self, "_h", None) is not None and self._h.value:
            self.lib.blsv_service_destroy(self._h)
            self._h = None

    def __enter__(self):
        return self

    def __exit__(self, *exc):
        self.close()

    def verify_partial(self, commits, n, msg, partial):
        cb = b"".join(bytes(c) for c in commits)
        ok, cls = ctypes.c_uint8(), ctypes.c_uint8()
        p = bytes(partial)
        rc = self.lib.blsv_service_verify_partial(self._h, _lib.buf(cb), len(commits), int(n), _lib.buf(msg), len(msg),
                                                  _lib.buf(p), len(p), ctypes.byref(ok), ctypes.byref(cls))
        if rc != 0:
            raise EngineError(rc, "blsv_service_verify_partial failed")
        return bool(ok.value), cls.value

    def prepare_partial(self, commits, n, msg, partial):
        cb = _lib.buf(b"".join(bytes(c) for c in commits))
        mb, pb = _lib.buf(msg), _lib.buf(bytes(partial))
        t, ml, pl = len(commits), len(msg), len(partial)
        ok, cls = ctypes.c_uint8(), ctypes.c_uint8()
        f, h, pok, pcls = self.lib.blsv_service_verify_partial, self._h, ctypes.byref(ok), ctypes.byref(cls)

        def call():
            rc = f(h, cb, t, n, mb, ml, pb, pl, pok, pcls)
            if rc != 0:
                raise EngineError(rc, "blsv_service_verify_partial failed")
            return bool(ok.value), cls.value

        return call

    def verify_recovered(self, pk48, msg, sig96):
        ok, cls = ctypes.c_uint8(), ctypes.c_uint8()
        rc = self.lib.blsv_service_verify_recovered(self._h, _lib.buf(pk48), _lib.buf(msg), len(msg), _lib.buf(sig96),
                                                    ctypes.byref(ok), ctypes.byref(cls))
        if rc != 0:
            raise EngineError(rc, "blsv_service_verify_recovered failed")
        return bool(ok.value), cls.value

    def test_limits(self, chunk=0, lat_max=(1 << 64) - 1, arena_entries=0):
        n = ctypes.c_uint64()
        rc = self.lib.blsv_test_service_limits(self._h, int(chunk), int(lat_max), int(arena_entries), ctypes.byref(n))
        if rc != 0:
            raise EngineError(rc, "blsv_test_service_limits failed")
        return n.value

    def stats(self):
        a, b, c = ctypes.c_uint64(), ctypes.c_uint64(), ctypes.c_uint64()
        self.lib.blsv_service_stats(self._h, ctypes.byref(a), ctypes.byref(b), ctypes.byref(c))
        return a.value, b.value, c.value


def limbs_of(v, n=12):
    return [(v >> (32 * i)) & 0xFFFFFFFF for i in range(n)]


def int_of(limbs):
    return sum(int(x) << (32 * i) for i, x in enumerate(limbs))
```

### include/blsverify_testing.h

```cpp
#ifndef DRAND_AMD_BLSVERIFY_TESTING_H
#define DRAND_AMD_BLSVERIFY_TESTING_H

#include "blsverify.h"

#ifdef __cplusplus
extern "C" {
#endif

int blsv_test_fp_mul(blsv_ctx* ctx, const uint32_t* a, const uint32_t* b, size_t n, uint32_t* out);

int blsv_test_pairing(blsv_ctx* ctx, const uint32_t* p, const uint32_t* q, size_t n, uint32_t* out_f);

int blsv_test_final_exp(blsv_ctx* ctx, const uint32_t* f, size_t n, uint32_t* out_pipeline, uint32_t* out_ref);

int blsv_test_tail_split(blsv_ctx* ctx, size_t q);

int blsv_test_op(blsv_ctx* ctx, const char* name, const uint32_t* in, size_t n, uint32_t* out);
int blsv_test_op_info(int index, const char** name, int* in_fp, int* out_fp, int* lanes);

int blsv_test_hash_to_g2(blsv_ctx* ctx, const uint8_t* msgs, const uint32_t* msg_lens, size_t n, uint32_t* out,
                         uint8_t* inf);

int blsv_test_generic_chains(blsv_ctx* ctx, int on);

int blsv_test_spec_stats(blsv_ctx* ctx, uint64_t* hits, uint64_t* misses);

int blsv_test_service_limits(blsv_service* svc, size_t chunk, size_t lat_max, size_t arena_entries,
                             uint64_t* sub_launches);

int blsv_profile_enable(blsv_ctx* ctx, int on);
int blsv_lat_trace(blsv_ctx* ctx, uint64_t* ticks, int n, double* ticks_per_us, int clear);
int blsv_lat_trace_enable(blsv_ctx* ctx, int on);
int blsv_profile_read(blsv_ctx* ctx, double* ms, uint64_t* launches, uint64_t* items, int nstages);
int blsv_test_lagrange(const uint32_t* idx, size_t t, uint32_t* out);

int blsv_test_rlc_seed(blsv_ctx* ctx, const uint8_t* seed32);
int blsv_test_rlc_sums(blsv_ctx* ctx, uint64_t first_round, const uint8_t* prev0, size_t prev0_len,
                       const uint8_t* sigs96, size_t n, uint8_t* out_a96, uint8_t* out_b96);

#ifdef __cplusplus
}
#endif

#endif
```

Baseline: 2.453 million beacons/s.

## Batch field inversions with Montgomery's trick in final-exp easy part and G2 affine conversion

Replaces per-item Fp inversions in the easy part of the final exponentiation and in hash-to-G2 Jacobian-to-affine conversion with Montgomery batch inversion. Each lane chains up to K items through a prefix product, does one fp_inv, then unwinds. Partial products and norms are parked in the output buffers between the two passes. Batching is used only above a size threshold, and it cuts the costly binary-GCD inversions at the price of extra multiplications, global-memory round trips and fewer active lanes.

```diff
diff --git a/drand_amd/_lib.py b/drand_amd/_lib.py
--- a/drand_amd/_lib.py
+++ b/drand_amd/_lib.py
@@ -80,7 +80,10 @@
     "blsv_test_pairing": (ctypes.c_int, [vp, u32p, u32p, sz, u32p]),
     "blsv_test_hash_to_g2": (ctypes.c_int, [vp, u8p, u32p, sz, u32p, u8p]),
     "blsv_test_final_exp": (ctypes.c_int, [vp, u32p, sz, u32p, u32p]),
+    "blsv_test_final_exp_cls": (ctypes.c_int, [vp, u32p, u8p, sz, u32p, u32p]),
+    "blsv_test_g2_affine": (ctypes.c_int, [vp, u32p, sz, u32p, u8p]),
     "blsv_test_tail_split": (ctypes.c_int, [vp, sz]),
+    "blsv_test_inv_batch": (ctypes.c_int, [vp, sz, sz]),
     "blsv_set_lat_max": (sz, [vp, sz]),
     "blsv_set_chunk": (sz, [vp, sz]),
     "blsv_workspace_bytes": (sz, [vp]),
diff --git a/drand_amd/csrc/blsverify.cpp b/drand_amd/csrc/blsverify.cpp
--- a/drand_amd/csrc/blsverify.cpp
+++ b/drand_amd/csrc/blsverify.cpp
@@ -116,6 +116,7 @@
   int cus = 0;
   if (e == hipSuccess) e = hipDeviceGetAttribute(&cus, hipDeviceAttributeMultiprocessorCount, device);
   c->tail_q_dev = c->tail_q = size_t(64) * 4 * (size_t)std::max(cus, 0);
+  c->inv_batch.round_lanes = c->tail_q_dev;
   if (e != hipSuccess) {
     fprintf(stderr, "blsv_create: %s\n", hipGetErrorString(e));
     blsv_destroy(c);
diff --git a/drand_amd/csrc/engine_ctx.h b/drand_amd/csrc/engine_ctx.h
--- a/drand_amd/csrc/engine_ctx.h
+++ b/drand_amd/csrc/engine_ctx.h
@@ -178,6 +178,7 @@
   size_t lat_max = std::min(lat_max_env(), chunk);
   uint64_t oom_halvings = 0;
   size_t tail_q_dev = 0, tail_q = 0;
+  blsk::InvBatch inv_batch;
   std::vector<ProfRec> recs;
   std::vector<hipEvent_t> event_pool;
   hipStream_t stream = nullptr;
diff --git a/drand_amd/csrc/fp.h b/drand_amd/csrc/fp.h
--- a/drand_amd/csrc/fp.h
+++ b/drand_amd/csrc/fp.h
@@ -779,6 +779,26 @@
 
 DI fp fp_inv(const fp& a) { return fp_from_u12(fp_inv_bingcd(fp_to_u12(a))); }
 
+DI fp fp_inv_chain_push(fp& acc, const fp& a) {
+  const fp pre = acc;
+  acc = fp_mul(acc, fp_select(fp_is_zero(a), fp_one(), a));
+  return pre;
+}
+DI fp fp_inv_chain_pop(fp& inv, const fp& a, const fp& pre) {
+  const bool z = fp_is_zero(a);
+  const fp r = fp_mul(inv, pre);
+  inv = fp_mul(inv, fp_select(z, fp_one(), a));
+  return fp_select(z, fp_zero(), r);
+}
+template <int K>
+DI void fp_inv_batch(fp (&a)[K]) {
+  fp pre[K];
+  fp acc = fp_one();
+  for (int k = 0; k < K; k++) pre[k] = fp_inv_chain_push(acc, a[k]);
+  fp inv = fp_inv(acc);
+  for (int k = K - 1; k >= 0; k--) a[k] = fp_inv_chain_pop(inv, a[k], pre[k]);
+}
+
 DI fp fp_sqrt_cand(const fp& a) { return fp_from_u12(fp_pow_sqrt(fp_to_u12(a))); }
 
 DI bool fp_is_square(const fp& a) {
diff --git a/drand_amd/csrc/host_internal.h b/drand_amd/csrc/host_internal.h
--- a/drand_amd/csrc/host_internal.h
+++ b/drand_amd/csrc/host_internal.h
@@ -58,12 +58,12 @@
 
 inline void hash_chained(blsv_ctx* c, const blsk::ChainedSrc& src, size_t base, size_t cnt, hipStream_t st) {
   const Staging w = staging(c);
-  blsk::launch_hash_chained(src, base, cnt, w.H, w.h_inf, w.HQ, st);
+  blsk::launch_hash_chained(src, base, cnt, w.H, w.h_inf, w.HQ, st, c->inv_batch);
 }
 inline void hash_messages(blsv_ctx* c, const uint8_t* d_msgs, const uint64_t* d_off, const uint32_t* d_len, size_t base,
                           size_t cnt, hipStream_t st) {
   const Staging w = staging(c);
-  blsk::launch_hash_messages(d_msgs, d_off + base, d_len + base, cnt, w.H, w.h_inf, w.HQ, st);
+  blsk::launch_hash_messages(d_msgs, d_off + base, d_len + base, cnt, w.H, w.h_inf, w.HQ, st, c->inv_batch);
 }
 inline void hash_uploaded(blsv_ctx* c, size_t base, size_t cnt, hipStream_t st) {
   hash_messages(c, c->in_msgs.as<uint8_t>(), c->in_off.as<uint64_t>(), c->in_len.as<uint32_t>(), base, cnt, st);
@@ -76,7 +76,8 @@
 inline void final_exp(blsv_ctx* c, size_t cnt, size_t base, size_t m, uint8_t* cls, hipStream_t st,
                       uint32_t* out = nullptr) {
   const Staging w = staging(c);
-  blsk::launch_final_exp(w.F, w.FW, cnt, base, m, cls, st, w.HQ + (base ? blsk::FEXP_PARK_WORDS(base) : 0), out);
+  blsk::launch_final_exp(w.F, w.FW, cnt, base, m, cls, st, w.HQ + (base ? blsk::FEXP_PARK_WORDS(base) : 0), out,
+                         c->inv_batch);
 }
 inline void final_exp(blsv_ctx* c, size_t cnt, uint8_t* cls, hipStream_t st, uint32_t* out = nullptr) {
   final_exp(c, cnt, 0, cnt, cls, st, out);
diff --git a/drand_amd/csrc/k_fexp.hip b/drand_amd/csrc/k_fexp.hip
--- a/drand_amd/csrc/k_fexp.hip
+++ b/drand_amd/csrc/k_fexp.hip
@@ -1,3 +1,5 @@
+#include <algorithm>
+
 #include "kcommon.h"
 
 namespace blsk {
@@ -6,6 +8,36 @@
   size_t i = (size_t)blockIdx.x * TPB + threadIdx.x;
   if (i >= m || cls[i] != REJ_OK) return;
   st_fp12(G, n, i, fexp_easy(ld_fp12(F, n, i)));
+}
+
+BLS_KERNEL(BLS_WPE_FEXP) k_fexp_easy_batch(const uint32_t* F, size_t n, size_t m, size_t L, int K, const uint8_t* cls,
+                                           uint32_t* G) {
+  const size_t j = (size_t)blockIdx.x * TPB + threadIdx.x;
+  if (j >= L) return;
+  fp acc = fp_one();
+#pragma unroll 1
+  for (int k = 0; k < K; k++) {
+    const size_t i = j + (size_t)k * L;
+    if (i >= m || cls[i] != REJ_OK) continue;
+    fp12_inv_part s;
+    const fp nrm = fp12_inv_norm(ld_fp12(F, n, i), s);
+    st_fp2(G, n, i, 0, s.t0);
+    st_fp2(G, n, i, 2, s.t1);
+    st_fp2(G, n, i, 4, s.t2);
+    st_fp2(G, n, i, 6, s.d);
+    st_fp(G, n, i, 8, nrm);
+    st_fp(G, n, i, 9, fp_inv_chain_push(acc, nrm));
+  }
+  fp inv = fp_inv(acc);
+#pragma unroll 1
+  for (int k = K - 1; k >= 0; k--) {
+    const size_t i = j + (size_t)k * L;
+    if (i >= m || cls[i] != REJ_OK) continue;
+    const fp12_inv_part s = {ld_fp2(G, n, i, 0), ld_fp2(G, n, i, 2), ld_fp2(G, n, i, 4), ld_fp2(G, n, i, 6)};
+    const fp ni = fp_inv_chain_pop(inv, ld_fp(G, n, i, 8), ld_fp(G, n, i, 9));
+    const fp12 f = ld_fp12(F, n, i);
+    st_fp12(G, n, i, fexp_easy_from_inv(f, fp12_inv_finish(f, s, ni)));
+  }
 }
 
 #ifndef BLS_WPE_FEXP_TRI
@@ -66,8 +98,15 @@
   }
 }
 
+constexpr size_t kFexpInvKMax = 16;
+static size_t fexp_batch_lanes(size_t m, size_t round_lanes) {
+  const size_t q = round_lanes ? round_lanes : 1;
+  const size_t rounds = (m + q * kFexpInvKMax - 1) / (q * kFexpInvKMax);
+  return std::min(m, rounds * q);
+}
+
 void launch_final_exp(uint32_t* F, uint32_t* W, size_t n, size_t base, size_t m, uint8_t* cls, hipStream_t st,
-                      uint32_t* park, uint32_t* out) {
+                      uint32_t* park, uint32_t* out, const InvBatch& ib) {
   if (!m) return;
   F += base;
   cls += base;
@@ -76,7 +115,12 @@
   uint32_t* B = G + n * F_WORDS;
   uint32_t* C = G + 2 * n * F_WORDS;
   const dim3 grid(grid_for(m)), blk(TPB);
-  hipLaunchKernelGGL(k_fexp_easy, grid, blk, 0, st, F, n, m, cls, G);
+  if (m >= ib.min_items) {
+    const size_t L = fexp_batch_lanes(m, ib.round_lanes);
+    hipLaunchKernelGGL(k_fexp_easy_batch, dim3(grid_for(L)), blk, 0, st, F, n, m, L, (int)((m + L - 1) / L), cls, G);
+  } else {
+    hipLaunchKernelGGL(k_fexp_easy, grid, blk, 0, st, F, n, m, cls, G);
+  }
   const dim3 tgrid((unsigned)((m + TRI_GROUPS - 1) / TRI_GROUPS));
   hipLaunchKernelGGL(k_fexp_tri<0>, tgrid, blk, 0, st, G, nullptr, nullptr, n, m, cls, F, park);
   hipLaunchKernelGGL(k_fexp_tri<1>, tgrid, blk, 0, st, F, nullptr, nullptr, n, m, cls, B, park);
diff --git a/drand_amd/csrc/k_hash.hip b/drand_amd/csrc/k_hash.hip
--- a/drand_amd/csrc/k_hash.hip
+++ b/drand_amd/csrc/k_hash.hip
@@ -198,12 +198,50 @@
   store_h(H, h_inf, cnt, i, load_jac(Q, cnt, i, 6));
 }
 
+#ifndef BLS_HASH_INV_K
+#define BLS_HASH_INV_K 8
+#endif
+template <int K>
+BLS_KERNEL(BLS_WPE_HASH_C) k_hash_affine_batch(const uint32_t* Q, size_t cnt, size_t L, uint32_t* H, uint8_t* h_inf) {
+  const size_t j = (size_t)blockIdx.x * TPB + threadIdx.x;
+  if (j >= L) return;
+  fp acc = fp_one();
+#pragma unroll 1
+  for (int k = 0; k < K; k++) {
+    const size_t i = j + (size_t)k * L;
+    if (i >= cnt) continue;
+    const fp nrm = fp2_norm(ld_fp2(Q, cnt, i, 10));
+    st_fp(H, cnt, i, 0, nrm);
+    st_fp(H, cnt, i, 1, fp_inv_chain_push(acc, nrm));
+  }
+  fp inv = fp_inv(acc);
+#pragma unroll 1
+  for (int k = K - 1; k >= 0; k--) {
+    const size_t i = j + (size_t)k * L;
+    if (i >= cnt) continue;
+    const fp ni = fp_inv_chain_pop(inv, ld_fp(H, cnt, i, 0), ld_fp(H, cnt, i, 1));
+    const g2j h = load_jac(Q, cnt, i, 6);
+    const fp2 zi = fp2_inv_from_norm(h.z, ni), zi2 = fp2_sqr(zi);
+    st_fp2(H, cnt, i, 0, fp2_mul(h.x, zi2));
+    st_fp2(H, cnt, i, 2, fp2_mul(h.y, fp2_mul(zi2, zi)));
+    h_inf[i] = jac_is_inf(h);
+  }
+}
+
 int g_generic_chains_all = 0;
-static void launch_hash_bc(uint32_t* Q, size_t cnt, uint32_t* H, uint8_t* h_inf, hipStream_t st) {
+void launch_hash_affine(const uint32_t* Q, size_t cnt, uint32_t* H, uint8_t* h_inf, hipStream_t st, bool batch) {
+  if (!cnt) return;
+  const size_t L = (cnt + BLS_HASH_INV_K - 1) / BLS_HASH_INV_K;
+  if (batch)
+    hipLaunchKernelGGL(k_hash_affine_batch<BLS_HASH_INV_K>, dim3(grid_for(L)), dim3(TPB), 0, st, Q, cnt, L, H, h_inf);
+  else
+    hipLaunchKernelGGL(k_hash_affine, dim3(grid_for(cnt)), dim3(TPB), 0, st, Q, cnt, H, h_inf);
+}
+static void launch_hash_bc(uint32_t* Q, size_t cnt, uint32_t* H, uint8_t* h_inf, hipStream_t st, const InvBatch& ib) {
   hipLaunchKernelGGL(k_hash_cofactor, dim3(grid_for(cnt)), dim3(TPB), 0, st, Q, cnt, h_inf);
   hipLaunchKernelGGL(k_hash_cofactor_generic, dim3(grid_for(cnt)), dim3(TPB), 0, st, Q, cnt, h_inf,
                      g_generic_chains_all);
-  hipLaunchKernelGGL(k_hash_affine, dim3(grid_for(cnt)), dim3(TPB), 0, st, Q, cnt, H, h_inf);
+  launch_hash_affine(Q, cnt, H, h_inf, st, cnt >= ib.min_items);
 }
 
 #ifndef BLS_HASH_SPLIT_MAX
@@ -212,18 +250,18 @@
 static inline dim3 hash_a_grid(size_t cnt, bool split) { return dim3((split ? 2u : 1u) * grid_for(cnt)); }
 
 void launch_hash_chained(const ChainedSrc& src, size_t base, size_t cnt, uint32_t* H, uint8_t* h_inf,
-                         uint32_t* Q, hipStream_t st) {
+                         uint32_t* Q, hipStream_t st, const InvBatch& ib) {
   if (!cnt) return;
   const bool split = cnt <= BLS_HASH_SPLIT_MAX;
   if (split)
     hipLaunchKernelGGL(k_hash_chained<true>, hash_a_grid(cnt, true), dim3(TPB), 0, st, src, base, cnt, Q);
   else
     hipLaunchKernelGGL(k_hash_chained<false>, hash_a_grid(cnt, false), dim3(TPB), 0, st, src, base, cnt, Q);
-  launch_hash_bc(Q, cnt, H, h_inf, st);
+  launch_hash_bc(Q, cnt, H, h_inf, st, ib);
 }
 
 void launch_hash_unchained(const uint64_t* rounds, uint64_t first_round, size_t base, size_t cnt, uint32_t* H,
-                           uint8_t* h_inf, uint32_t* Q, hipStream_t st) {
+                           uint8_t* h_inf, uint32_t* Q, hipStream_t st, const InvBatch& ib) {
   if (!cnt) return;
   const bool split = cnt <= BLS_HASH_SPLIT_MAX;
   if (split)
@@ -232,18 +270,18 @@
   else
     hipLaunchKernelGGL(k_hash_unchained<false>, hash_a_grid(cnt, false), dim3(TPB), 0, st, rounds, first_round, base,
                        cnt, Q);
-  launch_hash_bc(Q, cnt, H, h_inf, st);
+  launch_hash_bc(Q, cnt, H, h_inf, st, ib);
 }
 
 void launch_hash_messages(const uint8_t* msgs, const uint64_t* off, const uint32_t* len, size_t cnt, uint32_t* H,
-                          uint8_t* h_inf, uint32_t* Q, hipStream_t st) {
+                          uint8_t* h_inf, uint32_t* Q, hipStream_t st, const InvBatch& ib) {
   if (!cnt) return;
   const bool split = cnt <= BLS_HASH_SPLIT_MAX;
   if (split)
     hipLaunchKernelGGL(k_hash_messages<true>, hash_a_grid(cnt, true), dim3(TPB), 0, st, msgs, off, len, cnt, Q);
   else
     hipLaunchKernelGGL(k_hash_messages<false>, hash_a_grid(cnt, false), dim3(TPB), 0, st, msgs, off, len, cnt, Q);
-  launch_hash_bc(Q, cnt, H, h_inf, st);
-}
-
-}
+  launch_hash_bc(Q, cnt, H, h_inf, st, ib);
+}
+
+}
diff --git a/drand_amd/csrc/kernels.h b/drand_amd/csrc/kernels.h
--- a/drand_amd/csrc/kernels.h
+++ b/drand_amd/csrc/kernels.h
@@ -19,13 +19,19 @@
   uint64_t seg_phase;
 };
 
+constexpr size_t kInvBatchMin = 65536;
+struct InvBatch {
+  size_t min_items = kInvBatchMin;
+  size_t round_lanes = 65536;
+};
 constexpr int HQ_WORDS = 144;
 void launch_hash_chained(const ChainedSrc& src, size_t base, size_t cnt, uint32_t* H, uint8_t* h_inf,
-                         uint32_t* Q, hipStream_t st);
+                         uint32_t* Q, hipStream_t st, const InvBatch& ib = InvBatch());
 void launch_hash_unchained(const uint64_t* rounds, uint64_t first_round, size_t base, size_t cnt, uint32_t* H,
-                           uint8_t* h_inf, uint32_t* Q, hipStream_t st);
+                           uint8_t* h_inf, uint32_t* Q, hipStream_t st, const InvBatch& ib = InvBatch());
 void launch_hash_messages(const uint8_t* msgs, const uint64_t* off, const uint32_t* len, size_t cnt,
-                          uint32_t* H, uint8_t* h_inf, uint32_t* Q, hipStream_t st);
+                          uint32_t* H, uint8_t* h_inf, uint32_t* Q, hipStream_t st, const InvBatch& ib = InvBatch());
+void launch_hash_affine(const uint32_t* Q, size_t cnt, uint32_t* H, uint8_t* h_inf, hipStream_t st, bool batch);
 void launch_decompress_g2(const uint8_t* sigs, size_t stride, size_t offset, size_t base, size_t cnt, uint32_t* S,
                           uint8_t* s_inf, uint8_t* cls, hipStream_t st);
 constexpr int MILLER_LINE_WORDS = 68 * 2 * 6 * 12;
@@ -40,7 +46,7 @@
 constexpr size_t TRI_PARK_WORDS(size_t items) { return 48 * 64 * ((items + 20) / 21); }
 constexpr size_t FEXP_PARK_WORDS(size_t items) { return TRI_PARK_WORDS(items); }
 void launch_final_exp(uint32_t* F, uint32_t* W, size_t n, size_t base, size_t m, uint8_t* cls, hipStream_t st,
-                      uint32_t* park, uint32_t* out = nullptr);
+                      uint32_t* park, uint32_t* out = nullptr, const InvBatch& ib = InvBatch());
 void launch_finish(const uint8_t* cls, size_t base, size_t cnt, uint64_t* bitmap, unsigned long long* first_bad,
                    uint64_t label0, hipStream_t st);
 
@@ -108,6 +114,7 @@
 void launch_test_fp_mul(const uint32_t* a, const uint32_t* b, size_t cnt, uint32_t* out, hipStream_t st);
 void launch_test_pairing(const uint32_t* p_tab, const uint32_t* q_aff, size_t cnt, uint32_t* out_f, hipStream_t st);
 void launch_test_unpack_g2(const uint32_t* H, size_t cnt, uint32_t* out, hipStream_t st);
+void launch_test_pack_jac(const uint32_t* in, size_t cnt, uint32_t* Q, hipStream_t st);
 void launch_test_pack_fp12(const uint32_t* f, size_t cnt, uint32_t* F, hipStream_t st);
 void launch_test_unpack_fp12(const uint32_t* F, size_t cnt, uint32_t* out, hipStream_t st);
 void launch_test_final_exp_ref(const uint32_t* F, size_t cnt, uint32_t* out, hipStream_t st);
diff --git a/drand_amd/csrc/pairing.h b/drand_amd/csrc/pairing.h
--- a/drand_amd/csrc/pairing.h
+++ b/drand_amd/csrc/pairing.h
@@ -274,10 +274,11 @@
   return fp12_conj(f);
 }
 
-DI fp12 fexp_easy(const fp12& f) {
-  fp12 t = fp12_mul(fp12_conj(f), fp12_inv(f));
+DI fp12 fexp_easy_from_inv(const fp12& f, const fp12& fi) {
+  fp12 t = fp12_mul(fp12_conj(f), fi);
   return fp12_mul(fp12_frob2(t), t);
 }
+DI fp12 fexp_easy(const fp12& f) { return fexp_easy_from_inv(f, fp12_inv(f)); }
 
 template <typename Load>
 DI fp12 fp12_pow_x_abs_reload(Load load) {
diff --git a/drand_amd/csrc/testhooks.cpp b/drand_amd/csrc/testhooks.cpp
--- a/drand_amd/csrc/testhooks.cpp
+++ b/drand_amd/csrc/testhooks.cpp
@@ -83,6 +83,13 @@
   return BLSV_OK;
 }
 
+int blsv_test_inv_batch(blsv_ctx* c, size_t min_items, size_t round_lanes) {
+  if (!c) return BLSV_EINVAL;
+  c->inv_batch.min_items = min_items == SIZE_MAX ? blsk::kInvBatchMin : min_items;
+  c->inv_batch.round_lanes = round_lanes == SIZE_MAX ? c->tail_q_dev : round_lanes;
+  return BLSV_OK;
+}
+
 int blsv_test_generic_chains(blsv_ctx* c, int on) {
   if (!c) return BLSV_EINVAL;
   blsk::g_generic_chains_all = on != 0;
@@ -148,6 +155,11 @@
 }
 
 int blsv_test_final_exp(blsv_ctx* c, const uint32_t* f, size_t n, uint32_t* out_pipeline, uint32_t* out_ref) {
+  return blsv_test_final_exp_cls(c, f, nullptr, n, out_pipeline, out_ref);
+}
+
+int blsv_test_final_exp_cls(blsv_ctx* c, const uint32_t* f, const uint8_t* cls, size_t n, uint32_t* out_pipeline,
+                            uint32_t* out_ref) {
   if (!c || (n && (!f || !out_pipeline || !out_ref))) return BLSV_EINVAL;
   if (n > kMaxChunk) return BLSV_EINVAL;
   (void)hipSetDevice(c->device);
@@ -161,7 +173,12 @@
   HIPCHK(c, dref.ensure(n * 576));
   const Staging w = staging(c);
   HIPCHK(c, hipMemcpyAsync(din.p, f, n * 576, hipMemcpyHostToDevice, c->stream));
-  HIPCHK(c, hipMemsetAsync(w.cls, 0, n, c->stream));
+  if (cls) {
+    HIPCHK(c, h2d(c, w.cls, cls, n));
+    HIPCHK(c, hipMemsetAsync(dout.p, 0, n * 576, c->stream));
+  } else {
+    HIPCHK(c, hipMemsetAsync(w.cls, 0, n, c->stream));
+  }
   blsk::launch_test_pack_fp12(din.as<uint32_t>(), n, w.F, c->stream);
   blsk::launch_test_final_exp_ref(w.F, n, dref.as<uint32_t>(), c->stream);
   const size_t mn = tail_split_main(n, c->tail_q);
@@ -232,4 +249,27 @@
   return BLSV_OK;
 }
 
-}
+int blsv_test_g2_affine(blsv_ctx* c, const uint32_t* jac, size_t n, uint32_t* out, uint8_t* inf) {
+  if (!c || (n && (!jac || !out || !inf))) return BLSV_EINVAL;
+  if (n > kMaxChunk) return BLSV_EINVAL;
+  if (!n) return BLSV_OK;
+  (void)hipSetDevice(c->device);
+  int rc = ensure_workspace(c, n);
+  if (rc) return rc;
+  if (n > c->cap) return fail(c, BLSV_EINVAL, "test_g2_affine: more than the context chunk");
+  DBuf din, dout;
+  HIPCHK(c, din.ensure(n * 288));
+  HIPCHK(c, dout.ensure(n * 192));
+  const Staging w = staging(c);
+  HIPCHK(c, hipMemcpyAsync(din.p, jac, n * 288, hipMemcpyHostToDevice, c->stream));
+  blsk::launch_test_pack_jac(din.as<uint32_t>(), n, w.HQ, c->stream);
+  blsk::launch_hash_affine(w.HQ, n, w.H, w.h_inf, c->stream, n >= c->inv_batch.min_items);
+  blsk::launch_test_unpack_g2(w.H, n, dout.as<uint32_t>(), c->stream);
+  HIPCHK(c, hipGetLastError());
+  HIPCHK(c, hipMemcpyAsync(out, dout.p, n * 192, hipMemcpyDeviceToHost, c->stream));
+  HIPCHK(c, hipMemcpyAsync(inf, w.h_inf, n, hipMemcpyDeviceToHost, c->stream));
+  HIPCHK(c, hipStreamSynchronize(c->stream));
+  return BLSV_OK;
+}
+
+}
diff --git a/drand_amd/csrc/tlock.cpp b/drand_amd/csrc/tlock.cpp
--- a/drand_amd/csrc/tlock.cpp
+++ b/drand_amd/csrc/tlock.cpp
@@ -49,7 +49,7 @@
   }
   {
     StageTimer tm(c, ST_FEXP, cnt, st);
-    blsk::launch_final_exp(w.F, w.FW, cnt, 0, cnt, w.cls, st, w.LN, w.HQ);
+    blsk::launch_final_exp(w.F, w.FW, cnt, 0, cnt, w.cls, st, w.LN, w.HQ, c->inv_batch);
   }
   blsk::launch_tlock_encode(w.HQ, ucls, cnt, d_out, st);
   if (d_cls_out) HIPCHK(c, hipMemcpyAsync(d_cls_out, ucls, cnt, hipMemcpyDeviceToDevice, st));
diff --git a/drand_amd/csrc/tower.h b/drand_amd/csrc/tower.h
--- a/drand_amd/csrc/tower.h
+++ b/drand_amd/csrc/tower.h
@@ -269,6 +269,15 @@
 }
 
 DI fp fp2_norm(const fp2& a) { return fp_add(fp_sqr(a.c0), fp_sqr(a.c1)); }
+
+DI fp2 fp2_inv_from_norm(const fp2& z, const fp& ni) { return {fp_mul(z.c0, ni), fp_neg(fp_mul(z.c1, ni))}; }
+template <int K>
+DI void fp2_inv_batch(fp2 (&a)[K]) {
+  fp n[K];
+  for (int k = 0; k < K; k++) n[k] = fp2_norm(a[k]);
+  fp_inv_batch<K>(n);
+  for (int k = 0; k < K; k++) a[k] = fp2_inv_from_norm(a[k], n[k]);
+}
 
 DI fp fp_norm_root(const fp& n, bool& is_sq) {
   fp s = fp_mul(fp_pow_sqrt_inv(n), n);
@@ -576,6 +585,23 @@
   return {fp6_mul(a.c0, di), fp6_neg(fp6_mul(a.c1, di))};
 }
 
+struct fp12_inv_part {
+  fp2 t0, t1, t2, d;
+};
+DI fp fp12_inv_norm(const fp12& a, fp12_inv_part& s) {
+  const fp6 e = fp6_sub(fp6_sqr(a.c0), fp6_mul_v(fp6_sqr(a.c1)));
+  s.t0 = fp2_sub(fp2_sqr(e.c0), fp2_mul_xi(fp2_mul(e.c1, e.c2)));
+  s.t1 = fp2_sub(fp2_mul_xi(fp2_sqr(e.c2)), fp2_mul(e.c0, e.c1));
+  s.t2 = fp2_sub(fp2_sqr(e.c1), fp2_mul(e.c0, e.c2));
+  s.d = fp2_add(fp2_mul(e.c0, s.t0), fp2_mul_xi(fp2_add(fp2_mul(e.c2, s.t1), fp2_mul(e.c1, s.t2))));
+  return fp2_norm(s.d);
+}
+DI fp12 fp12_inv_finish(const fp12& a, const fp12_inv_part& s, const fp& ni) {
+  const fp2 di = fp2_inv_from_norm(s.d, ni);
+  const fp6 ei = {fp2_mul(s.t0, di), fp2_mul(s.t1, di), fp2_mul(s.t2, di)};
+  return {fp6_mul(a.c0, ei), fp6_neg(fp6_mul(a.c1, ei))};
+}
+
 DI fp12 fp12_frob(const fp12& a) {
   fp12 r;
   r.c0.c0 = fp2_conj(a.c0.c0);
diff --git a/drand_amd/csrc/verify.cpp b/drand_amd/csrc/verify.cpp
--- a/drand_amd/csrc/verify.cpp
+++ b/drand_amd/csrc/verify.cpp
@@ -411,7 +411,7 @@
       c, n, sig, pk,
       [&](size_t base, size_t cnt, hipStream_t st) {
         const Staging w = staging(c);
-        blsk::launch_hash_unchained(d_rounds, first_round, base, cnt, w.H, w.h_inf, w.HQ, st);
+        blsk::launch_hash_unchained(d_rounds, first_round, base, cnt, w.H, w.h_inf, w.HQ, st, c->inv_batch);
       },
       [&](uint8_t* cls) { blsk::launch_lat_unchained(d_rounds, first_round, sig.d, 0, n, pk.tab, pk.inf, cls, c->stream); },
       randomized, first_round, rounds, ok_bitmap, first_bad, reject_class);
diff --git a/drand_amd/engine.py b/drand_amd/engine.py
--- a/drand_amd/engine.py
+++ b/drand_amd/engine.py
@@ -487,16 +487,34 @@
         self._check(self.lib.blsv_test_pairing(self._h, Pp, Q, n, O))
         return list(O)[:n * 144]
 
-    def test_final_exp(self, f_words):
+    def test_final_exp(self, f_words, cls=None):
         n = len(f_words) // 144
         Fw = (ctypes.c_uint32 * max(len(f_words), 1))(*f_words)
         A = (ctypes.c_uint32 * max(n * 144, 1))()
         B = (ctypes.c_uint32 * max(n * 144, 1))()
-        self._check(self.lib.blsv_test_final_exp(self._h, Fw, n, A, B))
+        if cls is None:
+            self._check(self.lib.blsv_test_final_exp(self._h, Fw, n, A, B))
+        else:
+            if len(cls) != n:
+                raise ValueError("one class byte per item")
+            self._check(self.lib.blsv_test_final_exp_cls(self._h, Fw, _lib.buf(bytes(cls)), n, A, B))
         return list(A)[:n * 144], list(B)[:n * 144]
+
+    def test_g2_affine(self, jac_words):
+        n = len(jac_words) // 72
+        J = (ctypes.c_uint32 * max(len(jac_words), 1))(*jac_words)
+        O = (ctypes.c_uint32 * max(n * 48, 1))()
+        inf = _lib.out_buf(n)
+        self._check(self.lib.blsv_test_g2_affine(self._h, J, n, O, inf))
+        return list(O)[:n * 48], list(inf)[:n]
 
     def test_tail_split(self, q):
         self._check(self.lib.blsv_test_tail_split(self._h, ctypes.c_size_t(-1).value if q is None else int(q)))
+
+    def test_inv_batch(self, min_items=None, round_lanes=None):
+        none = ctypes.c_size_t(-1).value
+        self._check(self.lib.blsv_test_inv_batch(self._h, none if min_items is None else int(min_items),
+                                                 none if round_lanes is None else int(round_lanes)))
 
     def test_hash_to_g2(self, msgs):
         n = len(msgs)
diff --git a/include/blsverify_testing.h b/include/blsverify_testing.h
--- a/include/blsverify_testing.h
+++ b/include/blsverify_testing.h
@@ -12,11 +12,17 @@
 int blsv_test_pairing(blsv_ctx* ctx, const uint32_t* p, const uint32_t* q, size_t n, uint32_t* out_f);
 
 int blsv_test_final_exp(blsv_ctx* ctx, const uint32_t* f, size_t n, uint32_t* out_pipeline, uint32_t* out_ref);
+int blsv_test_final_exp_cls(blsv_ctx* ctx, const uint32_t* f, const uint8_t* cls, size_t n, uint32_t* out_pipeline,
+                            uint32_t* out_ref);
 
 int blsv_test_tail_split(blsv_ctx* ctx, size_t q);
 
+int blsv_test_inv_batch(blsv_ctx* ctx, size_t min_items, size_t round_lanes);
+
 int blsv_test_op(blsv_ctx* ctx, const char* name, const uint32_t* in, size_t n, uint32_t* out);
 int blsv_test_op_info(int index, const char** name, int* in_fp, int* out_fp, int* lanes);
+
+int blsv_test_g2_affine(blsv_ctx* ctx, const uint32_t* jac, size_t n, uint32_t* out, uint8_t* inf);
 
 int blsv_test_hash_to_g2(blsv_ctx* ctx, const uint8_t* msgs, const uint32_t* msg_lens, size_t n, uint32_t* out,
                          uint8_t* inf);
```

Result: no change. 2.465 million beacons/s (median of 6 runs) (+0.5%).
